# Quantum-Chemistry-Group-BNU/PyNQS

Measured on AMD Instinct MI355X. Metric: local energies/sec (whole node), higher is better.
Workload: dtype f64

## Files before the change

include/pynqs_amd.h:

```cpp
#ifndef PYNQS_AMD_H
#define PYNQS_AMD_H

#include <stdint.h>

#ifdef __cplusplus
extern "C" {
#endif

#define PYNQS_ABI_VERSION 1

#define PYNQS_OK 0
#define PYNQS_EINVAL (-1)
#define PYNQS_ELAUNCH (-2)
#define PYNQS_ELENGTH (-3)
#define PYNQS_EOVERFLOW (-4)

#define PYNQS_F32 0
#define PYNQS_F64 1

#define PYNQS_MAX_SORB_LEN 3
#define PYNQS_MAX_SORB 192
#define PYNQS_MAX_NELE 120
#define PYNQS_MAX_NVIR 120

int pynqs_abi_version(void);
const char *pynqs_last_error(void);

int64_t pynqs_num_sd(int sorb, int noA, int noB);

int pynqs_check_sorb(int sorb, int nele);

int pynqs_comb_hij_fused(const uint64_t *bra, int64_t nbatch, int sorb, int nele, int noA, int noB,
                         const void *h1e, const void *h2e, int dtype, uint64_t *comb, void *hmat,
                         void *stream);

int pynqs_comb(const uint64_t *bra, int64_t nbatch, int sorb, int noA, int noB, uint64_t *comb,
               double *comb_pm1, void *stream);

int pynqs_hij(const uint64_t *bra, int64_t n, const uint64_t *ket, int64_t m, int ket_is_3d,
              const void *h1e, const void *h2e, int dtype, int sorb, int nele, void *hmat, void *stream);

int pynqs_onv_to_pm1(const uint64_t *bra, int64_t n, int sorb, int dtype, void *out, void *stream);

int pynqs_pm01_to_onv(const uint8_t *occ, int64_t n, int sorb, uint64_t *out, void *stream);

int pynqs_wavefunction_lut(const uint64_t *keys, int64_t nkeys, const uint64_t *onv, int64_t n, int sorb,
                           int64_t *idx, uint8_t *mask, void *stream);

int pynqs_spin_flip_rand(const uint64_t *bra, int64_t n, int sorb, int noA, int noB, uint64_t seed,
                         uint64_t offset, uint64_t *out, void *stream);

int64_t pynqs_plan_bytes(int sorb, int dtype);
int pynqs_plan_build(const void *h1e, const void *h2e, int sorb, int dtype, void *plan, void *stream);

int pynqs_comb_hij_fused_plan(const uint64_t *bra, int64_t nbatch, int sorb, int nele, int noA, int noB,
                              const void *plan, int dtype, uint64_t *comb, void *hmat, void *stream);

int pynqs_eloc_sample_space(const uint64_t *bra, int64_t nbatch, int sorb, int nele, int noA, int noB,
                            const void *plan, const uint64_t *keys, int64_t nkeys, const double *wf,
                            int wf_is_complex, double *eloc, double *psi0, void *stream);

int64_t pynqs_hash_bytes(int64_t nkeys, int sorb);
int pynqs_hash_build(const uint64_t *keys, int64_t nkeys, int sorb, void *table, void *stream);
int pynqs_hash_lookup(const void *table, int64_t nkeys, const uint64_t *onv, int64_t n, int sorb, int64_t *idx,
                      uint8_t *mask, void *stream);
int pynqs_eloc_sample_space_hash(const uint64_t *bra, int64_t nbatch, int sorb, int nele, int noA, int noB,
                                 const void *plan, const void *table, int64_t nkeys, const double *wf,
                                 int wf_is_complex, double *eloc, double *psi0, void *stream);

int pynqs_eloc_sample_space_flip(const uint64_t *bra, int64_t nbatch, int sorb, int nele, int noA, int noB,
                                 const void *plan, const uint64_t *keys, int64_t nkeys, const double *wf,
                                 int wf_is_complex, const double *psi0, double *out, void *stream);
int pynqs_eloc_sample_space_hash_flip(const uint64_t *bra, int64_t nbatch, int sorb, int nele, int noA, int noB,
                                      const void *plan, const void *table, int64_t nkeys, const double *wf,
                                      int wf_is_complex, const double *psi0, double *out, void *stream);

int pynqs_eloc_sample_space_keys(const uint64_t *bra, int64_t nbatch, int sorb, int nele, int noA, int noB, const void *plan,
                                 const uint64_t *keys, int64_t nkeys, const double *wf, int wf_is_complex, int flip, double *eloc,
                                 double *psi0, void *stream);

int64_t pynqs_keys_index_bytes(int64_t nkeys, int sorb);
int64_t pynqs_keys_index_workspace(int64_t nkeys, int sorb);
int pynqs_keys_index_build(const uint64_t *keys, int64_t nkeys, int sorb, void *index, void *workspace, void *stream);
int pynqs_keys_index_density(const void *index, int64_t nkeys, int sorb, uint64_t *sum_sq, void *stream);
int pynqs_eloc_sample_space_indexed(const uint64_t *bra, int64_t nbatch, int sorb, int nele, int noA, int noB, const void *plan,
                                    const uint64_t *keys, int64_t nkeys, const void *index, const double *wf, int wf_is_complex,
                                    int flip, double *eloc, double *psi0, void *stream);

int pynqs_eloc_sample_space_form(int64_t nbatch, int sorb, int nele, int noA, int noB, int64_t nkeys, int hash, int64_t out[8]);
int pynqs_eloc_sample_space_keys_form(int64_t nbatch, int sorb, int64_t nkeys, int indexed, int64_t out[3]);

int64_t pynqs_unique_workspace(int64_t n);
int pynqs_unique_first(const uint64_t *onv, int64_t n, int sorb, void *workspace, int32_t *first, void *stream);

int pynqs_eloc_rbm_supported(int sorb, int nele, int noA, int noB, int nhidden);
int pynqs_eloc_rbm_form(int64_t nbatch, int sorb, int nele, int noA, int noB, int nhidden, int green);
int64_t pynqs_rbm_table_bytes(int sorb, int nhidden);
int pynqs_rbm_table_build(const double *weights, const double *hidden_bias, const double *visible_bias, int sorb,
                          int nhidden, void *table, void *stream);
int pynqs_eloc_rbm(const uint64_t *bra, int64_t nbatch, int sorb, int nele, int noA, int noB, const void *plan,
                   const void *rbm_table, int nhidden, double *eloc, double *psi, void *stream);
#define PYNQS_RBM_REAL 0
#define PYNQS_RBM_TANH 1
#define PYNQS_RBM_PHASE 2
int pynqs_eloc_rbm_flavour(const uint64_t *bra, int64_t nbatch, int sorb, int nele, int noA, int noB, const void *plan,
                           const void *rbm_table, int nhidden, int flavour, double *eloc, double *psi, void *stream);

int pynqs_eloc_rbm_flip_supported(int sorb, int nele, int noA, int noB, int nhidden);
int pynqs_eloc_rbm_flip_form(int64_t nbatch, int sorb, int nele, int noA, int noB, int nhidden);
int pynqs_eloc_rbm_signed(const uint64_t *bra, int64_t nbatch, int sorb, int nele, int noA, int noB, const void *plan,
                          const void *rbm_table, int nhidden, int flavour, double *eloc, double *psi, void *stream);
int pynqs_eloc_rbm_flip(const uint64_t *bra, int64_t nbatch, int sorb, int nele, int noA, int noB, const void *plan,
                        const void *rbm_table, const void *rbm_table_mirror, int nhidden, int flavour, double eta, double extra_norm,
                        const double *extra_norm_dev, double *eloc, double *psi, double *work, void *stream);

int pynqs_eloc_crbm_supported(int sorb, int nele, int noA, int noB, int nhidden);
int pynqs_eloc_crbm_form(int64_t nbatch, int sorb, int nele, int noA, int noB, int nhidden);
int64_t pynqs_crbm_table_bytes(int sorb, int nhidden);
int pynqs_crbm_table_build(const double *weights, const double *hidden_bias, const double *visible_bias, int sorb, int nhidden,
                           void *table, void *stream);
int pynqs_eloc_crbm(const uint64_t *bra, int64_t nbatch, int sorb, int nele, int noA, int noB, const void *plan,
                    const void *crbm_table, int nhidden, double log_scale, double *eloc, double *psi, void *stream);

int64_t pynqs_jastrow_table_bytes(int sorb);
int pynqs_jastrow_table_build(const double *jastrow, int sorb, void *table, void *stream);
int pynqs_eloc_jrbm_supported(int sorb, int nele, int noA, int noB, int nhidden);
int pynqs_eloc_jrbm_form(int64_t nbatch, int sorb, int nele, int noA, int noB, int nhidden);
int pynqs_eloc_jrbm(const uint64_t *bra, int64_t nbatch, int sorb, int nele, int noA, int noB, const void *plan,
                    const void *rbm_table, const void *jastrow_table, int nhidden, double *eloc, double *psi, void *stream);
int pynqs_eloc_jrbm_flip_supported(int sorb, int nele, int noA, int noB, int nhidden);
int pynqs_eloc_jrbm_flip_form(int64_t nbatch, int sorb, int nele, int noA, int noB, int nhidden);
int pynqs_eloc_jrbm_signed(const uint64_t *bra, int64_t nbatch, int sorb, int nele, int noA, int noB, const void *plan,
                           const void *rbm_table, const void *jastrow_table, int nhidden, double *eloc, double *psi, void *stream);
int pynqs_eloc_jrbm_flip(const uint64_t *bra, int64_t nbatch, int sorb, int nele, int noA, int noB, const void *plan,
                         const void *rbm_table, const void *jastrow_table, const void *rbm_table_mirror, const void *jastrow_table_mirror,
                         int nhidden, double eta, double extra_norm, const double *extra_norm_dev, double *eloc, double *psi, double *work,
                         void *stream);
int pynqs_jrbm_forward(const uint64_t *onv, int64_t n, int sorb, const double *weights, const double *hidden_bias,
                       const double *visible_bias, const double *jastrow, int nhidden, double *psi, void *stream);
int64_t pynqs_jastrow_grad_workspace(int64_t n, int sorb);
int pynqs_jastrow_grad(const uint64_t *onv, int64_t n, int sorb, const double *jastrow, const double *prob, const double *eloc,
                       const double *e_total, const double *pow, double *grad_jastrow, double *loss, void *workspace, void *stream);

int pynqs_gfmc_sample(const double *green, int64_t n, int64_t ncomb, const double *rand_num, const uint64_t *comb,
                      int sorb, int64_t *index, double *beta, uint64_t *x_new, void *stream);

int pynqs_green_rbm(const uint64_t *bra, int64_t nbatch, int sorb, int nele, int noA, int noB, const void *plan,
                    const void *rbm_table, int nhidden, int flavour, double lambda, double *eloc, double *psi, double *green,
                    uint8_t *clamped, void *stream);
int pynqs_gfmc_sample_rank(const double *green, int64_t n, const double *rand_num, const uint64_t *bra, int sorb, int nele,
                           int noA, int noB, int64_t *index, double *beta, uint64_t *x_new, void *stream);
int pynqs_green_jrbm(const uint64_t *bra, int64_t nbatch, int sorb, int nele, int noA, int noB, const void *plan,
                     const void *rbm_table, const void *jastrow_table, int nhidden, double lambda, double *eloc, double *psi,
                     double *green, uint8_t *clamped, void *stream);

int64_t pynqs_moments_workspace(void);
int pynqs_stats_finish(const double *moments, double inv_world, double counts, double *out5, void *stream);
int pynqs_weighted_moments(const double *x, int is_complex, const double *prob, int64_t n, void *workspace, void *stream);
int pynqs_weighted_moments_finish(const double *x, int is_complex, const double *prob, int64_t n, void *workspace, double inv_world,
                                  double counts, double *out5, void *stream);

int64_t pynqs_reduce_tiles(int64_t nbatch, int sorb, int nele, int noA, int noB);
int pynqs_reduce_count(const uint64_t *bra, int64_t nbatch, int sorb, int nele, int noA, int noB,
                       const void *plan, int dtype, double eps, uint32_t *tile_counts, void *stream);
int pynqs_reduce_emit(const uint64_t *bra, int64_t nbatch, int sorb, int nele, int noA, int noB,
                      const void *plan, int dtype, double eps, const int64_t *tile_offsets, int32_t *kept_col,
                      uint64_t *kept_onv, void *kept_h, void *stream);

int pynqs_reduce_count_sums(const uint64_t *bra, int64_t nbatch, int sorb, int nele, int noA, int noB,
                            const void *plan, int dtype, double eps, uint32_t *tile_counts, double *tile_sums,
                            void *stream);
int pynqs_reduce_sample(const uint64_t *bra, int64_t nbatch, int sorb, int nele, int noA, int noB, const void *plan,
                        int dtype, double eps, const int32_t *tile_draws, const int64_t *sample_offsets,
                        const double *walker_scale, uint64_t seed, int32_t *s_col, uint64_t *s_onv, void *s_h,
                        void *stream);

typedef struct pynqs_reduce_io {
  int64_t cap_doubles;
  int64_t cap_unique;
  int64_t dedup_slots;
  int32_t *rec_col;
  void *rec_w;
  uint64_t *rec_onv;
  int32_t *rec_link;
  int32_t *seg_count;
  int32_t *srec_col;
  void *srec_w;
  uint64_t *srec_onv;
  int32_t *srec_link;
  double *row_sum;
  void *dedup_table;
  uint64_t *uniq_onv;
  void *uniq_pm1;
  int32_t pm1_dtype;
  int32_t lut_is_hash;
  const void *lut_table;
  int64_t lut_nkeys;
  int32_t *counters;
  const uint64_t *seed_dev;
  void *row_cache;
  int32_t *uniq_parent;
  void *tile_scratch;
  int64_t tile_scratch_bytes;
  float *row_f32;
} pynqs_reduce_io;
int pynqs_reduce_onepass_geometry(int64_t nbatch, int sorb, int nele, int noA, int noB, int eps_sample, int64_t *out4);
int64_t pynqs_reduce_onepass_tile_scratch_bytes(int64_t nbatch, int sorb, int nele, int noA, int noB, int eps_sample);
int pynqs_reduce_onepass_list_capacity(int64_t nbatch, int sorb, int nele, int noA, int noB, int dtype, int eps_sample,
                                       int with_row_cache, int without_table, int64_t *cap_doubles);
int pynqs_reduce_onepass_wants_row_f32(int64_t nbatch, int sorb, int nele, int noA, int noB, int dtype, int eps_sample, int64_t cap_doubles,
                                       int with_tile_scratch ,
                                       int without_table );
int64_t pynqs_reduce_onepass_row_f32_elements(int64_t nbatch, int sorb, int nele, int noA, int noB);
int pynqs_reduce_onepass(const uint64_t *bra, int64_t nbatch, int sorb, int nele, int noA, int noB, const void *plan,
                         int dtype, double eps, int eps_sample, uint64_t seed, const pynqs_reduce_io *io, void *stream);
int pynqs_reduce_contract(int64_t nbatch, int sorb, int nele, int noA, int noB, int dtype, int eps_sample,
                          const pynqs_reduce_io *io, const double *psi_unique, const double *psi_table, int psi_is_complex,
                          int divide, double *eloc, double *psi_x, void *stream);

#define PYNQS_RBM_COMPLEX 4
int pynqs_rbm_forward(const uint64_t *onv, int64_t n, int sorb, const double *weights, const double *hidden_bias,
                      const double *visible_bias, int nhidden, int flavour, double *psi, void *stream);

int64_t pynqs_rbm_children_table_bytes(int64_t nwalkers, int sorb, int nhidden, int flavour);
int pynqs_rbm_children_prepare(const uint64_t *walkers, int64_t nwalkers, int sorb, const double *weights, const double *hidden_bias,
                               const double *visible_bias, int nhidden, int flavour, void *table, void *stream);
int pynqs_rbm_forward_children(const uint64_t *onv, int64_t n, const int32_t *count_dev, const int32_t *parent,
                               const uint64_t *walkers, int64_t nwalkers, const void *table, int sorb, const double *weights,
                               const double *hidden_bias, const double *visible_bias, int nhidden, int flavour, double *psi,
                               void *stream);
int pynqs_rbm_forward_children_supported(int sorb, int nhidden, int flavour);
int pynqs_rbm_children_prepare_stamped(const uint64_t *walkers, int64_t nwalkers, int sorb, const double *weights,
                                       const double *hidden_bias, const double *visible_bias, int nhidden, int flavour, uint64_t stamp,
                                       void *table, void *stream);
int pynqs_rbm_forward_children_stamped(const uint64_t *onv, int64_t n, const int32_t *count_dev, const int32_t *parent,
                                       const uint64_t *walkers, int64_t nwalkers, const void *table, int sorb, const double *weights,
                                       const double *hidden_bias, const double *visible_bias, int nhidden, int flavour, uint64_t stamp,
                                       double *psi, void *stream);

int64_t pynqs_rbm_grad_workspace(int64_t n, int sorb, int nhidden, int flavour);
int pynqs_rbm_grad(const uint64_t *onv, int64_t n, int sorb, const double *weights, const double *hidden_bias,
                   const double *visible_bias, int nhidden, int flavour, const double *prob, const double *eloc,
                   int eloc_is_complex, const double *e_total, const double *pow, double *grad_weights,
                   double *grad_hidden_bias, double *grad_visible_bias, double *loss, void *workspace, void *stream);
int pynqs_rbm_grad_loss(const uint64_t *onv, int64_t n, int sorb, const double *weights, const double *hidden_bias,
                        const double *visible_bias, int nhidden, int flavour, const double *prob, const double *eloc,
                        int eloc_is_complex, const double *e_total, const double *pow, double *grad_weights,
                        double *grad_hidden_bias, double *grad_visible_bias, double *loss, double *loss_copy, void *workspace,
                        void *stream);

#define PYNQS_SR_RHO 0
#define PYNQS_SR_RHS2 1
#define PYNQS_SR_DONE 2
#define PYNQS_SR_ITER 3
#define PYNQS_SR_TRUE2 4
#define PYNQS_SR_PAP 5
#define PYNQS_SR_CONVERGED 6
#define PYNQS_SR_BREAKDOWN 7
#define PYNQS_SR_NSCALARS 8
#define PYNQS_SR_CG_INIT 0
#define PYNQS_SR_CG_STEP 1
#define PYNQS_SR_CG_RESIDUAL 2
int64_t pynqs_rbm_sr_workspace(int64_t n, int sorb, int nhidden, int flavour);
int pynqs_rbm_sr_prepare(const uint64_t *onv, int64_t n, int sorb, const double *weights, const double *hidden_bias, int nhidden,
                         int flavour, const double *prob, void *workspace, double *obar, void *stream);
int pynqs_rbm_sr_matvec(const uint64_t *onv, int64_t n, int sorb, int nhidden, int flavour, const double *prob, const void *workspace,
                        const double *obar, const double *v, double *y, void *stream);
int pynqs_rbm_sr_cg_step(int mode, int64_t np, double *y, const double *rhs, double *d, double *r, double *p, double *scalars,
                         double inv_world, double diag_shift, double tol, void *stream);
int64_t pynqs_jrbm_sr_workspace(int64_t n, int sorb, int nhidden);
int pynqs_jrbm_sr_prepare(const uint64_t *onv, int64_t n, int sorb, const double *weights, const double *hidden_bias, int nhidden,
                          const double *prob, void *workspace, double *obar, void *stream);
int pynqs_jrbm_sr_matvec(const uint64_t *onv, int64_t n, int sorb, int nhidden, const double *prob, const void *workspace,
                         const double *obar, const double *v, double *y, void *stream);

#define PYNQS_MCMC_ACCEPT_KEY 0x243F6A8885A308D3ull
int pynqs_mcmc_rbm_supported(int sorb, int nhidden, int flavour);
int pynqs_mcmc_rbm(uint64_t *states, int64_t nchains, int sorb, int noA, int noB, const void *table, int nhidden, int flavour,
                   uint64_t seed, uint64_t chain_base, uint64_t t0, int nsteps, int every, uint64_t *records, int64_t *n_accept,
                   double *lnpsi, void *stream);
int pynqs_mcmc_jrbm_supported(int sorb, int nhidden);
int pynqs_mcmc_jrbm_form(int sorb, int nhidden);
int pynqs_mcmc_jrbm(uint64_t *states, int64_t nchains, int sorb, int noA, int noB, const void *rbm_table, const void *jastrow_table,
                    int nhidden, uint64_t seed, uint64_t chain_base, uint64_t t0, int nsteps, int every, uint64_t *records,
                    int64_t *n_accept, double *lnpsi, void *stream);
int pynqs_mcmc_accept(uint64_t *states, double *psi, const uint64_t *proposals, const double *psi_proposals, int64_t nchains,
                      int sorb, int is_complex, uint64_t seed, uint64_t chain_base, uint64_t t, uint64_t *record_row,
                      int64_t *n_accept, void *stream);

int pynqs_rdm_scatter(const uint64_t *bra, int64_t nbatch, int sorb, int nele, int noA, int noB, const double *w, const double *ratio,
                      int is_complex, double *rdm1, double *rdm2, void *stream);
int pynqs_rdm_rbm_supported(int sorb, int nele, int noA, int noB, int nhidden);
int64_t pynqs_rdm_rbm_workspace(int64_t nbatch, int sorb, int nhidden);
int pynqs_rdm_rbm(const uint64_t *bra, int64_t nbatch, int sorb, int nele, int noA, int noB, const double *w, const void *rbm_table,
                  int nhidden, void *workspace, double *rdm1, double *rdm2, void *stream);
int pynqs_rdm_jrbm_supported(int sorb, int nele, int noA, int noB, int nhidden);
int64_t pynqs_rdm_jrbm_workspace(int64_t nbatch, int sorb, int nhidden);
int pynqs_rdm_jrbm(const uint64_t *bra, int64_t nbatch, int sorb, int nele, int noA, int noB, const double *w, const void *rbm_table,
                   const void *jastrow_table, int nhidden, void *workspace, double *rdm1, double *rdm2, void *stream);

#ifdef __cplusplus
}
#endif
#endif
```

pynqs_amd/_native.py:

```python
from __future__ import annotations

import ctypes as C
import os

_HERE = os.path.dirname(os.path.abspath(__file__))
LIB_PATH = os.environ.get("PYNQS_AMD_LIB") or os.path.join(_HERE, "csrc", "libpynqs_amd.so")

PYNQS_F32, PYNQS_F64 = 0, 1
RBM_REAL, RBM_TANH, RBM_PHASE, RBM_COMPLEX = 0, 1, 2, 4
OK, EINVAL, ELAUNCH, ELENGTH, EOVERFLOW = 0, -1, -2, -3, -4

_i64, _int, _vp, _dbl = C.c_int64, C.c_int, C.c_void_p, C.c_double

SIGNATURES = {
    "pynqs_abi_version": (_int, []),
    "pynqs_last_error": (C.c_char_p, []),
    "pynqs_num_sd": (_i64, [_int, _int, _int]),
    "pynqs_check_sorb": (_int, [_int, _int]),
    "pynqs_comb_hij_fused": (_int, [_vp, _i64, _int, _int, _int, _int, _vp, _vp, _int, _vp, _vp, _vp]),
    "pynqs_comb": (_int, [_vp, _i64, _int, _int, _int, _vp, _vp, _vp]),
    "pynqs_hij": (_int, [_vp, _i64, _vp, _i64, _int, _vp, _vp, _int, _int, _int, _vp, _vp]),
    "pynqs_onv_to_pm1": (_int, [_vp, _i64, _int, _int, _vp, _vp]),
    "pynqs_pm01_to_onv": (_int, [_vp, _i64, _int, _vp, _vp]),
    "pynqs_wavefunction_lut": (_int, [_vp, _i64, _vp, _i64, _int, _vp, _vp, _vp]),
    "pynqs_spin_flip_rand": (_int, [_vp, _i64, _int, _int, _int, C.c_uint64, C.c_uint64, _vp, _vp]),
    "pynqs_plan_bytes": (_i64, [_int, _int]),
    "pynqs_plan_build": (_int, [_vp, _vp, _int, _int, _vp, _vp]),
    "pynqs_comb_hij_fused_plan": (_int, [_vp, _i64, _int, _int, _int, _int, _vp, _int, _vp, _vp, _vp]),
    "pynqs_eloc_sample_space": (_int, [_vp, _i64, _int, _int, _int, _int, _vp, _vp, _i64, _vp, _int, _vp, _vp, _vp]),
    "pynqs_hash_bytes": (_i64, [_i64, _int]),
    "pynqs_hash_build": (_int, [_vp, _i64, _int, _vp, _vp]),
    "pynqs_hash_lookup": (_int, [_vp, _i64, _vp, _i64, _int, _vp, _vp, _vp]),
    "pynqs_unique_workspace": (_i64, [_i64]),
    "pynqs_unique_first": (_int, [_vp, _i64, _int, _vp, _vp, _vp]),
    "pynqs_eloc_sample_space_hash": (_int, [_vp, _i64, _int, _int, _int, _int, _vp, _vp, _i64, _vp, _int, _vp, _vp, _vp]),
    "pynqs_eloc_sample_space_flip": (_int, [_vp, _i64, _int, _int, _int, _int, _vp, _vp, _i64, _vp, _int, _vp, _vp, _vp]),
    "pynqs_eloc_sample_space_hash_flip": (_int, [_vp, _i64, _int, _int, _int, _int, _vp, _vp, _i64, _vp, _int, _vp, _vp, _vp]),
    "pynqs_eloc_sample_space_keys": (_int, [_vp, _i64, _int, _int, _int, _int, _vp, _vp, _i64, _vp, _int, _int, _vp, _vp, _vp]),
    "pynqs_keys_index_bytes": (_i64, [_i64, _int]),
    "pynqs_keys_index_workspace": (_i64, [_i64, _int]),
    "pynqs_keys_index_build": (_int, [_vp, _i64, _int, _vp, _vp, _vp]),
    "pynqs_keys_index_density": (_int, [_vp, _i64, _int, _vp, _vp]),
    "pynqs_eloc_sample_space_indexed": (_int, [_vp, _i64, _int, _int, _int, _int, _vp, _vp, _i64, _vp, _vp, _int, _int, _vp, _vp, _vp]),
    "pynqs_eloc_sample_space_form": (_int, [_i64, _int, _int, _int, _int, _i64, _int, C.POINTER(_i64)]),
    "pynqs_eloc_sample_space_keys_form": (_int, [_i64, _int, _i64, _int, C.POINTER(_i64)]),
    "pynqs_eloc_rbm_supported": (_int, [_int, _int, _int, _int, _int]),
    "pynqs_eloc_rbm_form": (_int, [_i64, _int, _int, _int, _int, _int, _int]),
    "pynqs_rbm_table_bytes": (_i64, [_int, _int]),
    "pynqs_rbm_table_build": (_int, [_vp, _vp, _vp, _int, _int, _vp, _vp]),
    "pynqs_eloc_rbm": (_int, [_vp, _i64, _int, _int, _int, _int, _vp, _vp, _int, _vp, _vp, _vp]),
    "pynqs_eloc_rbm_flavour": (_int, [_vp, _i64, _int, _int, _int, _int, _vp, _vp, _int, _int, _vp, _vp, _vp]),
    "pynqs_eloc_rbm_flip_supported": (_int, [_int, _int, _int, _int, _int]),
    "pynqs_eloc_rbm_flip_form": (_int, [_i64, _int, _int, _int, _int, _int]),
    "pynqs_eloc_rbm_signed": (_int, [_vp, _i64, _int, _int, _int, _int, _vp, _vp, _int, _int, _vp, _vp, _vp]),
    "pynqs_eloc_rbm_flip": (_int, [_vp, _i64, _int, _int, _int, _int, _vp, _vp, _vp, _int, _int, _dbl, _dbl, _vp, _vp, _vp, _vp, _vp]),
    "pynqs_eloc_crbm_supported": (_int, [_int, _int, _int, _int, _int]),
    "pynqs_eloc_crbm_form": (_int, [_i64, _int, _int, _int, _int, _int]),
    "pynqs_crbm_table_bytes": (_i64, [_int, _int]),
    "pynqs_crbm_table_build": (_int, [_vp, _vp, _vp, _int, _int, _vp, _vp]),
    "pynqs_eloc_crbm": (_int, [_vp, _i64, _int, _int, _int, _int, _vp, _vp, _int, _dbl, _vp, _vp, _vp]),
    "pynqs_gfmc_sample": (_int, [_vp, _i64, _i64, _vp, _vp, _int, _vp, _vp, _vp, _vp]),
    "pynqs_green_rbm": (_int, [_vp, _i64, _int, _int, _int, _int, _vp, _vp, _int, _int, _dbl, _vp, _vp, _vp, _vp, _vp]),
    "pynqs_gfmc_sample_rank": (_int, [_vp, _i64, _vp, _vp, _int, _int, _int, _int, _vp, _vp, _vp, _vp]),
    "pynqs_moments_workspace": (_i64, []),
    "pynqs_stats_finish": (_int, [_vp, _dbl, _dbl, _vp, _vp]),
    "pynqs_weighted_moments": (_int, [_vp, _int, _vp, _i64, _vp, _vp]),
    "pynqs_weighted_moments_finish": (_int, [_vp, _int, _vp, _i64, _vp, _dbl, _dbl, _vp, _vp]),
    "pynqs_reduce_tiles": (_i64, [_i64, _int, _int, _int, _int]),
    "pynqs_reduce_count": (_int, [_vp, _i64, _int, _int, _int, _int, _vp, _int, _dbl, _vp, _vp]),
    "pynqs_reduce_count_sums": (_int, [_vp, _i64, _int, _int, _int, _int, _vp, _int, _dbl, _vp, _vp, _vp]),
    "pynqs_reduce_sample": (_int, [_vp, _i64, _int, _int, _int, _int, _vp, _int, _dbl, _vp, _vp, _vp, C.c_uint64, _vp, _vp, _vp, _vp]),
    "pynqs_reduce_emit": (_int, [_vp, _i64, _int, _int, _int, _int, _vp, _int, _dbl, _vp, _vp, _vp, _vp, _vp]),
}



class ReduceIO(C.Structure):
    _fields_ = [("cap_doubles", _i64), ("cap_unique", _i64), ("dedup_slots", _i64),
                ("rec_col", _vp), ("rec_w", _vp), ("rec_onv", _vp), ("rec_link", _vp), ("seg_count", _vp),
                ("srec_col", _vp), ("srec_w", _vp), ("srec_onv", _vp), ("srec_link", _vp), ("row_sum", _vp),
                ("dedup_table", _vp), ("uniq_onv", _vp), ("uniq_pm1", _vp), ("pm1_dtype", C.c_int32), ("lut_is_hash", C.c_int32),
                ("lut_table", _vp), ("lut_nkeys", _i64), ("counters", _vp), ("seed_dev", _vp), ("row_cache", _vp), ("uniq_parent", _vp),
                ("tile_scratch", _vp), ("tile_scratch_bytes", _i64), ("row_f32", _vp)]


SIGNATURES.update({
    "pynqs_reduce_onepass_geometry": (_int, [_i64, _int, _int, _int, _int, _int, C.POINTER(_i64)]),
    "pynqs_reduce_onepass_tile_scratch_bytes": (_i64, [_i64, _int, _int, _int, _int, _int]),
    "pynqs_reduce_onepass_list_capacity": (_int, [_i64, _int, _int, _int, _int, _int, _int, _int, _int, C.POINTER(_i64)]),
    "pynqs_reduce_onepass_wants_row_f32": (_int, [_i64, _int, _int, _int, _int, _int, _int, _i64, _int, _int]),
    "pynqs_reduce_onepass_row_f32_elements": (_i64, [_i64, _int, _int, _int, _int]),
    "pynqs_reduce_onepass": (_int, [_vp, _i64, _int, _int, _int, _int, _vp, _int, _dbl, _int, C.c_uint64, C.POINTER(ReduceIO), _vp]),
    "pynqs_rbm_forward": (_int, [_vp, _i64, _int, _vp, _vp, _vp, _int, _int, _vp, _vp]),
    "pynqs_rbm_children_table_bytes": (_i64, [_i64, _int, _int, _int]),
    "pynqs_rbm_children_prepare": (_int, [_vp, _i64, _int, _vp, _vp, _vp, _int, _int, _vp, _vp]),
    "pynqs_rbm_forward_children": (_int, [_vp, _i64, _vp, _vp, _vp, _i64, _vp, _int, _vp, _vp, _vp, _int, _int, _vp, _vp]),
    "pynqs_rbm_forward_children_supported": (_int, [_int, _int, _int]),
    "pynqs_rbm_children_prepare_stamped": (_int, [_vp, _i64, _int, _vp, _vp, _vp, _int, _int, C.c_uint64, _vp, _vp]),
    "pynqs_rbm_forward_children_stamped": (_int, [_vp, _i64, _vp, _vp, _vp, _i64, _vp, _int, _vp, _vp, _vp, _int, _int, C.c_uint64, _vp, _vp]),
    "pynqs_rbm_grad_workspace": (_i64, [_i64, _int, _int, _int]),
    "pynqs_rbm_grad": (_int, [_vp, _i64, _int, _vp, _vp, _vp, _int, _int, _vp, _vp, _int, _vp, _vp, _vp, _vp, _vp, _vp, _vp, _vp]),
    "pynqs_rbm_grad_loss": (_int, [_vp, _i64, _int, _vp, _vp, _vp, _int, _int, _vp, _vp, _int, _vp, _vp, _vp, _vp, _vp, _vp, _vp, _vp, _vp]),
    "pynqs_reduce_contract": (_int, [_i64, _int, _int, _int, _int, _int, _int, C.POINTER(ReduceIO), _vp, _vp, _int, _int, _vp, _vp, _vp]),    "pynqs_mcmc_rbm_supported": (_int, [_int, _int, _int]),
    "pynqs_mcmc_rbm": (_int, [_vp, _i64, _int, _int, _int, _vp, _int, _int, C.c_uint64, C.c_uint64, C.c_uint64, _int, _int, _vp, _vp, _vp, _vp]),
    "pynqs_rbm_sr_workspace": (_i64, [_i64, _int, _int, _int]),
    "pynqs_rbm_sr_prepare": (_int, [_vp, _i64, _int, _vp, _vp, _int, _int, _vp, _vp, _vp, _vp]),
    "pynqs_rbm_sr_matvec": (_int, [_vp, _i64, _int, _int, _int, _vp, _vp, _vp, _vp, _vp, _vp]),
    "pynqs_rbm_sr_cg_step": (_int, [_int, _i64, _vp, _vp, _vp, _vp, _vp, _vp, _dbl, _dbl, _dbl, _vp]),
    "pynqs_jrbm_sr_workspace": (_i64, [_i64, _int, _int]),
    "pynqs_jrbm_sr_prepare": (_int, [_vp, _i64, _int, _vp, _vp, _int, _vp, _vp, _vp, _vp]),
    "pynqs_jrbm_sr_matvec": (_int, [_vp, _i64, _int, _int, _vp, _vp, _vp, _vp, _vp, _vp]),
    "pynqs_mcmc_accept": (_int, [_vp, _vp, _vp, _vp, _i64, _int, _int, C.c_uint64, C.c_uint64, C.c_uint64, _vp, _vp, _vp]),
    "pynqs_rdm_scatter": (_int, [_vp, _i64, _int, _int, _int, _int, _vp, _vp, _int, _vp, _vp, _vp]),
    "pynqs_rdm_rbm_supported": (_int, [_int, _int, _int, _int, _int]),
    "pynqs_rdm_rbm_workspace": (_i64, [_i64, _int, _int]),
    "pynqs_rdm_rbm": (_int, [_vp, _i64, _int, _int, _int, _int, _vp, _vp, _int, _vp, _vp, _vp, _vp]),
    "pynqs_rdm_jrbm_supported": (_int, [_int, _int, _int, _int, _int]),
    "pynqs_rdm_jrbm_workspace": (_i64, [_i64, _int, _int]),
    "pynqs_rdm_jrbm": (_int, [_vp, _i64, _int, _int, _int, _int, _vp, _vp, _vp, _int, _vp, _vp, _vp, _vp]),
    "pynqs_jastrow_table_bytes": (_i64, [_int]),
    "pynqs_jastrow_table_build": (_int, [_vp, _int, _vp, _vp]),
    "pynqs_eloc_jrbm_supported": (_int, [_int, _int, _int, _int, _int]),
    "pynqs_eloc_jrbm_form": (_int, [_i64, _int, _int, _int, _int, _int]),
    "pynqs_eloc_jrbm": (_int, [_vp, _i64, _int, _int, _int, _int, _vp, _vp, _vp, _int, _vp, _vp, _vp]),
    "pynqs_eloc_jrbm_flip_supported": (_int, [_int, _int, _int, _int, _int]),
    "pynqs_eloc_jrbm_flip_form": (_int, [_i64, _int, _int, _int, _int, _int]),
    "pynqs_eloc_jrbm_signed": (_int, [_vp, _i64, _int, _int, _int, _int, _vp, _vp, _vp, _int, _vp, _vp, _vp]),
    "pynqs_eloc_jrbm_flip": (_int, [_vp, _i64, _int, _int, _int, _int, _vp, _vp, _vp, _vp, _vp, _int, _dbl, _dbl, _vp, _vp, _vp, _vp, _vp]),
    "pynqs_green_jrbm": (_int, [_vp, _i64, _int, _int, _int, _int, _vp, _vp, _vp, _int, _dbl, _vp, _vp, _vp, _vp, _vp]),
    "pynqs_jrbm_forward": (_int, [_vp, _i64, _int, _vp, _vp, _vp, _vp, _int, _vp, _vp]),
    "pynqs_jastrow_grad_workspace": (_i64, [_i64, _int]),
    "pynqs_mcmc_jrbm_supported": (_int, [_int, _int]),
    "pynqs_mcmc_jrbm_form": (_int, [_int, _int]),
    "pynqs_mcmc_jrbm": (_int, [_vp, _i64, _int, _int, _int, _vp, _vp, _int, C.c_uint64, C.c_uint64, C.c_uint64, _int, _int, _vp, _vp, _vp, _vp]),
    "pynqs_jastrow_grad": (_int, [_vp, _i64, _int, _vp, _vp, _vp, _vp, _vp, _vp, _vp, _vp, _vp]),
})

_lib = None


class NativeLibraryError(RuntimeError):
    pass


def lib() -> C.CDLL:
    global _lib
    if _lib is None:
        if not os.path.exists(LIB_PATH):
            raise NativeLibraryError(
                f"{LIB_PATH} not found: build the HIP extension first (python -c 'import __graft_entry__ as g; g.build()'). "
                "pynqs_amd has no CPU fallback."
            )
        try:
            l = C.CDLL(LIB_PATH)
        except OSError as e:
            raise NativeLibraryError(f"cannot load {LIB_PATH}: {e}") from e
        for name, (res, args) in SIGNATURES.items():
            f = getattr(l, name)
            f.restype = res
            f.argtypes = args
        if l.pynqs_abi_version() != 1:
            raise NativeLibraryError("libpynqs_amd.so ABI version mismatch")
        _lib = l
    return _lib


def check(rc: int, what: str) -> None:
    if rc == OK:
        return
    msg = lib().pynqs_last_error().decode(errors="replace")
    if rc == ELENGTH:
        raise ValueError(msg)
    if rc == EOVERFLOW:
        raise OverflowError(msg)
    raise RuntimeError(f"{what}: {msg} (code {rc})")
```

pynqs_amd/csrc/kernels_gfmc.hip:

```cpp
#include "detcore.h"
#include "launch.h"

namespace pynqs {

constexpr int kGfmcMaxTiles = 1024;

__device__ __forceinline__ double wave_incl_scan(double v, int lane) {
#pragma unroll
  for (int d = 1; d < 64; d <<= 1) {
    const double o = __shfl_up(v, d);
    if (lane >= d) v += o;
  }
  return v;
}

template <int LEN, bool FROM_RANK>
__global__ __launch_bounds__(kBlock) void gfmc_sample_kernel(const double *__restrict__ gk, int64_t m, uint32_t tile, uint32_t ntiles,
                                                             const double *__restrict__ rnd, const uint64_t *__restrict__ comb, SDParams p,
                                                             int64_t *__restrict__ index, double *__restrict__ beta,
                                                             uint64_t *__restrict__ x_new) {
  __shared__ double tsum[kGfmcMaxTiles];
  __shared__ double s_target, s_before;
  __shared__ uint32_t s_tile;
  const int64_t walker = blockIdx.x;
  const int tid = threadIdx.x, lane = tid & 63, wave = tid >> 6;
  const double *__restrict__ row = gk + walker * m;
  for (uint32_t t = wave; t < ntiles; t += kBlock / 64) {
    const int64_t c0 = (int64_t)t * tile, c1 = min(c0 + (int64_t)tile, m);
    double acc = 0.0;
    for (int64_t c = c0 + lane; c < c1; c += 64) acc += row[c];
#pragma unroll
    for (int d = 32; d > 0; d >>= 1) acc += __shfl_xor(acc, d);
    if (lane == 0) tsum[t] = acc;
  }
  __syncthreads();
  if (wave == 0) {
    constexpr int kPer = kGfmcMaxTiles / 64;
    double loc[kPer], s = 0.0;
#pragma unroll
    for (int i = 0; i < kPer; ++i) {
      const uint32_t t = lane * kPer + i;
      loc[i] = t < ntiles ? tsum[t] : 0.0;
      s += loc[i];
    }
    const double incl = wave_incl_scan(s, lane);
    const double total = __shfl(incl, 63);
    const double target = rnd[walker] * total;
    const double lower = __shfl_up(incl, 1);
    double before = lane ? lower : 0.0;
    uint32_t mine = 0xffffffffu, last = 0xffffffffu;
    double mine_before = 0.0, last_before = 0.0;
#pragma unroll
    for (int i = 0; i < kPer; ++i) {
      const uint32_t t = lane * kPer + i;
      if (loc[i] > 0.0) {
        if (mine == 0xffffffffu && before + loc[i] >= target) { mine = t; mine_before = before; }
        last = t; last_before = before;
      }
      before += loc[i];
    }
    const uint64_t have = __ballot(mine != 0xffffffffu);
    const uint64_t any = __ballot(last != 0xffffffffu);
    const int src = have ? __ffsll((long long)have) - 1 : any ? 63 - __clzll((long long)any) : 0;
    if (lane == src) {
      s_tile = !(target > 0.0) ? 0xffffffffu : have ? mine : any ? last : 0xffffffffu;
      s_before = have ? mine_before : last_before;
      s_target = target;
    }
    if (lane == 0) beta[walker] = total;
  }
  __syncthreads();
  if (wave == 0) {
    const uint32_t t = s_tile;
    const double target = s_target;
    double run = s_before;
    const int64_t c0 = (int64_t)t * tile, c1 = min(c0 + (int64_t)tile, m);
    int64_t found = -1, last_pos = -1;
    if (t == 0xffffffffu) found = 0;
    for (int64_t c = c0; c < c1 && found < 0; c += 64) {
      const double v = c + lane < c1 ? row[c + lane] : 0.0;
      const double incl = wave_incl_scan(v, lane) + run;
      const uint64_t pos = __ballot(v > 0.0);
      const uint64_t hit = pos & __ballot(incl >= target);
      if (hit) found = c + __ffsll((long long)hit) - 1;
      if (pos) last_pos = c + 63 - __clzll((long long)pos);
      run = __shfl(incl, 63);
    }
    if (found < 0) found = last_pos >= 0 ? last_pos : 0;
    if (lane == 0) index[walker] = found;
    if constexpr (FROM_RANK) {
      if (lane == 0) {
        uint64_t x[LEN];
#pragma unroll
        for (int i = 0; i < LEN; ++i) x[i] = comb[walker * LEN + i];
        if (found > 0) excite_by_rank<LEN>(x, (uint32_t)(found - 1), p);
#pragma unroll
        for (int i = 0; i < LEN; ++i) x_new[walker * LEN + i] = x[i];
      }
    } else {
      if (lane < LEN) x_new[walker * LEN + lane] = comb[(walker * m + found) * LEN + lane];
    }
  }
}

}

using namespace pynqs;

template <bool FROM_RANK>
static int gfmc_sample_impl(const double *green, int64_t n, int64_t ncomb, const double *rand_num, const uint64_t *comb, int sorb,
                            const SDParams &p, int64_t *index, double *beta, uint64_t *x_new, void *stream) {
  pynqs::DeviceScope device_scope_(green);
  if (n < 0 || ncomb < 1 || sorb < 1 || sorb > kMaxSorb) return set_error(PYNQS_EINVAL, "bad n / ncomb / sorb");
  if (n == 0) return PYNQS_OK;
  if (!green || !rand_num || !comb || !index || !beta || !x_new) return set_error(PYNQS_EINVAL, "null pointer");
  if (n > 0x7fffffffll) return set_error(PYNQS_EINVAL, "n too large for one launch");
  uint32_t tile = 256;
  while ((ncomb + tile - 1) / tile > kGfmcMaxTiles) tile *= 2;
  const uint32_t ntiles = (uint32_t)((ncomb + tile - 1) / tile);
  const int len = (sorb - 1) / 64 + 1;
  hipStream_t st = (hipStream_t)stream;
  DISPATCH_LEN(len, hipLaunchKernelGGL((gfmc_sample_kernel<LEN, FROM_RANK>), dim3((uint32_t)n), dim3(kBlock), 0, st, green, ncomb, tile, ntiles,
                                       rand_num, comb, p, index, beta, x_new));
  return check_launch("gfmc_sample");
}

extern "C" int pynqs_gfmc_sample(const double *green, int64_t n, int64_t ncomb, const double *rand_num, const uint64_t *comb, int sorb,
                                 int64_t *index, double *beta, uint64_t *x_new, void *stream) {
  SDParams p = {};
  return gfmc_sample_impl<false>(green, n, ncomb, rand_num, comb, sorb, p, index, beta, x_new, stream);
}

extern "C" int pynqs_gfmc_sample_rank(const double *green, int64_t n, const double *rand_num, const uint64_t *bra, int sorb, int nele,
                                      int noA, int noB, int64_t *index, double *beta, uint64_t *x_new, void *stream) {
  SDParams p;
  if (!make_sd_params(sorb, nele, noA, noB, &p)) return set_error(PYNQS_EINVAL, "bad sorb/noA/noB");
  return gfmc_sample_impl<true>(green, n, (int64_t)p.nsd + 1, rand_num, bra, sorb, p, index, beta, x_new, stream);
}

namespace pynqs {

constexpr int kMomentBlocks = 128;

__device__ __forceinline__ void stats_finish(const double *m, double inv_world, double counts, double *__restrict__ out) {
  const double re = m[0] * inv_world, im = m[1] * inv_world, m2 = m[2] * inv_world, ps = m[3] * inv_world;
  double var = m2 - (re * re + im * im) * (2.0 - ps);
  var = var > 0.0 ? var : 0.0;
  const double sd = sqrt(var);
  out[0] = re; out[1] = im; out[2] = var; out[3] = sd; out[4] = sd / sqrt(counts);
}

template <bool CPLX, bool FINISH>
__global__ __launch_bounds__(kBlock) void moments_kernel(const double *__restrict__ x, const double *__restrict__ prob, int64_t n,
                                                         double *__restrict__ out, unsigned int *__restrict__ done, double inv_world,
                                                         double counts, double *__restrict__ out5) {
  __shared__ double red[4][kBlock / 64];
  __shared__ bool last;
  const int tid = threadIdx.x, lane = tid & 63, wave = tid >> 6;
  double s[4] = {0.0, 0.0, 0.0, 0.0};
  for (int64_t i = (int64_t)blockIdx.x * kBlock + tid; i < n; i += (int64_t)gridDim.x * kBlock) {
    const double p = prob[i];
    const double re = CPLX ? x[2 * i] : x[i], im = CPLX ? x[2 * i + 1] : 0.0;
    s[0] += p * re; s[1] += p * im; s[2] += p * (re * re + im * im); s[3] += p;
  }
#pragma unroll
  for (int k = 0; k < 4; ++k) {
#pragma unroll
    for (int d = 32; d > 0; d >>= 1) s[k] += __shfl_xor(s[k], d);
    if (lane == 0) red[k][wave] = s[k];
  }
  __syncthreads();
  if (tid < 4) {
    double t = 0.0;
    for (int w = 0; w < kBlock / 64; ++w) t += red[tid][w];
    out[4 * (1 + blockIdx.x) + tid] = t;
  }
  __threadfence();
  __syncthreads();
  if (tid == 0) last = atomicAdd(done, 1u) == gridDim.x - 1;
  __syncthreads();
  if (last) {
    __threadfence();
    if (tid < 4) {
      double t = 0.0;
      for (unsigned b = 0; b < gridDim.x; ++b) t += out[4 * (1 + b) + tid];
      out[tid] = t;
      if constexpr (FINISH) red[0][tid] = t;
    }
    if (tid == 0) *done = 0;
    if constexpr (FINISH) {
      __syncthreads();
      if (tid == 0) stats_finish(&red[0][0], inv_world, counts, out5);
    }
  }
}

__global__ void stats_finish_kernel(const double *__restrict__ m, double inv_world, double counts, double *__restrict__ out) {
  stats_finish(m, inv_world, counts, out);
}

}

extern "C" int pynqs_stats_finish(const double *moments, double inv_world, double counts, double *out5, void *stream) {
  pynqs::DeviceScope device_scope_(moments);
  if (!moments || !out5 || !(counts > 0.0)) return set_error(PYNQS_EINVAL, "bad arguments");
  hipLaunchKernelGGL(stats_finish_kernel, dim3(1), dim3(1), 0, (hipStream_t)stream, moments, inv_world, counts, out5);
  return check_launch("stats_finish");
}

extern "C" int64_t pynqs_moments_workspace(void) { return 8 * 4 * (pynqs::kMomentBlocks + 1) + 8; }

static int weighted_moments_launch(const double *x, int is_complex, const double *prob, int64_t n, void *workspace, bool finish, double inv_world,
                                   double counts, double *out5, void *stream) {
  pynqs::DeviceScope device_scope_(x);
  if (n < 0) return set_error(PYNQS_EINVAL, "bad n");
  if (!workspace || (n > 0 && (!x || !prob))) return set_error(PYNQS_EINVAL, "null pointer");
  if (finish && (!out5 || !(counts > 0.0))) return set_error(PYNQS_EINVAL, "bad arguments");
  double *out = (double *)workspace;
  unsigned int *done = (unsigned int *)(out + 4 * (kMomentBlocks + 1));
  int64_t blocks = (n + kBlock - 1) / kBlock;
  if (blocks > kMomentBlocks) blocks = kMomentBlocks;
  if (blocks < 1) blocks = 1;
  hipStream_t st = (hipStream_t)stream;
#define PYNQS_MK(C, F) \
  hipLaunchKernelGGL((moments_kernel<C, F>), dim3((uint32_t)blocks), dim3(kBlock), 0, st, x, prob, n, out, done, inv_world, counts, out5)
  if (finish) { if (is_complex) PYNQS_MK(true, true); else PYNQS_MK(false, true); }
  else { if (is_complex) PYNQS_MK(true, false); else PYNQS_MK(false, false); }
#undef PYNQS_MK
  return check_launch("weighted_moments");
}

extern "C" int pynqs_weighted_moments(const double *x, int is_complex, const double *prob, int64_t n, void *workspace, void *stream) {
  return weighted_moments_launch(x, is_complex, prob, n, workspace, false, 1.0, 1.0, nullptr, stream);
}

extern "C" int pynqs_weighted_moments_finish(const double *x, int is_complex, const double *prob, int64_t n, void *workspace, double inv_world,
                                             double counts, double *out5, void *stream) {
  return weighted_moments_launch(x, is_complex, prob, n, workspace, true, inv_world, counts, out5, stream);
}
```

pynqs_amd/csrc/kernels_rbm_grad.hip:

```cpp
#include "detcore.h"
#include "launch.h"
#include "rbm_math.h"

namespace pynqs {

constexpr int kGradWalkers = 32;
constexpr int kGradHidden = 32;

template <int LEN, bool CPLX, int B>
__global__ __launch_bounds__(B) void rbm_grad_partial_kernel(const uint64_t *__restrict__ onv, int64_t n, int sorb, int H,
                                                                  const double *__restrict__ W, const double *__restrict__ hb,
                                                                  const double *__restrict__ vb, const double *__restrict__ prob,
                                                                  const double *__restrict__ eloc, bool eloc_cplx,
                                                                  const double *__restrict__ e_total, const double *__restrict__ pw,
                                                                  double *__restrict__ partial, int64_t stride) {
  constexpr int C = CPLX ? 2 : 1;
  __shared__ uint64_t xs[kGradWalkers][LEN];
  __shared__ double tc[kGradWalkers][kGradHidden + 1][C];
  __shared__ double cf[kGradWalkers][C];
  constexpr int NQ = B / kGradWalkers;
  const int tid = threadIdx.x, w = tid % kGradWalkers, q = tid / kGradWalkers;
  const int64_t i = (int64_t)blockIdx.x * kGradWalkers + w;
  const bool valid = i < n;
  const int64_t row = valid ? i : n - 1;
  uint64_t ket[LEN];
#pragma unroll
  for (int k = 0; k < LEN; ++k) ket[k] = onv[row * LEN + k];
  double fr = 0.0, fi = 0.0;
  if (valid) {
    const double pr = prob[i], c = pw ? pw[i] : 1.0;
    const double er = eloc_cplx ? eloc[2 * i] : eloc[i], ei = eloc_cplx ? eloc[2 * i + 1] : 0.0;
    const double tr = e_total[0], ti = eloc_cplx ? e_total[1] : 0.0;
    fr = pr * (er - tr * c);
    fi = pr * (ei - ti * c);
  }
  if (q == 0) {
#pragma unroll
    for (int k = 0; k < LEN; ++k) xs[w][k] = ket[k];
    cf[w][0] = fr;
    if constexpr (CPLX) cf[w][1] = -fi;
  }
  double *__restrict__ out = partial + (int64_t)blockIdx.x * stride;
  double lre = 0.0, lim = 0.0;
  const int SP = sorb + 1;
  for (int h0 = 0; h0 < H; h0 += kGradHidden) {
    constexpr int HC = kGradHidden / NQ;
    double tr[HC], ti[HC];
#pragma unroll
    for (int j = 0; j < HC; ++j) {
      const int h = min(h0 + HC * q + j, H - 1);
      tr[j] = CPLX ? hb[2 * h] : hb[h];
      ti[j] = CPLX ? hb[2 * h + 1] : 0.0;
    }
    for (int o = 0; o < sorb; ++o) {
      const double x = pm1_of<LEN>(ket, o);
#pragma unroll
      for (int j = 0; j < HC; ++j) {
        const int h = min(h0 + HC * q + j, H - 1);
        if constexpr (CPLX) {
          tr[j] = fma(x, W[((size_t)h * sorb + o) * 2], tr[j]);
          ti[j] = fma(x, W[((size_t)h * sorb + o) * 2 + 1], ti[j]);
        } else {
          tr[j] = fma(x, W[(size_t)h * sorb + o], tr[j]);
        }
      }
    }
    if (h0) __syncthreads();
#pragma unroll
    for (int j = 0; j < HC; ++j) {
      const int hh = HC * q + j;
      const bool live = h0 + hh < H;
      const double ax = fabs(tr[j]), e = exp(-2.0 * ax), s = tr[j] < 0.0 ? -1.0 : 1.0;
      double yr, yi = 0.0;
      if constexpr (CPLX) {
        double sn, cs;
        sincos_mod(2.0 * ti[j], sn, cs);
        const double den = fma(2.0 * e, cs, fma(e, e, 1.0));
        yr = s * (1.0 - e * e) / den;
        yi = 2.0 * e * sn / den;
        if (live) {
          const double u = fma(e, cs, 1.0), v = -s * e * sn;
          lre += ax + 0.5 * log(u * u + v * v);
          lim += s * ti[j] + atan2(v, u);
        }
        tc[w][hh][0] = live ? yr * fr + yi * fi : 0.0;
        tc[w][hh][1] = live ? yi * fr - yr * fi : 0.0;
      } else {
        yr = s * (1.0 - e) / (1.0 + e);
        if (live) lre += ax + log1p(e);
        tc[w][hh][0] = live ? yr * fr : 0.0;
      }
    }
    __syncthreads();
    const int nout = min(kGradHidden, H - h0) * SP;
    for (int k = tid; k < nout; k += B) {
      const int hh = k / SP, o = k - hh * SP;
      double ar = 0.0, ai = 0.0;
      if (o < sorb) {
        const int word = o >> 6, bit = o & 63;
#pragma unroll 8
        for (int v = 0; v < kGradWalkers; ++v) {
          const bool up = (xs[v][word] >> bit) & 1ull;
          const double a = tc[v][hh][0];
          ar += up ? a : -a;
          if constexpr (CPLX) { const double b = tc[v][hh][1]; ai += up ? b : -b; }
        }
      } else {
#pragma unroll 8
        for (int v = 0; v < kGradWalkers; ++v) {
          ar += tc[v][hh][0];
          if constexpr (CPLX) ai += tc[v][hh][1];
        }
      }
      const int64_t at = (int64_t)(h0 + hh) * SP + o;
      out[C * at] = ar;
      if constexpr (CPLX) out[C * at + 1] = ai;
    }
  }
  const int64_t off_vb = (int64_t)H * SP;
  for (int o = tid; o < sorb; o += B) {
    const int word = o >> 6, bit = o & 63;
    double ar = 0.0, ai = 0.0;
#pragma unroll 4
    for (int v = 0; v < kGradWalkers; ++v) {
      const bool up = (xs[v][word] >> bit) & 1ull;
      ar += up ? cf[v][0] : -cf[v][0];
      if constexpr (CPLX) ai += up ? cf[v][1] : -cf[v][1];
    }
    out[C * (off_vb + o)] = ar;
    if constexpr (CPLX) out[C * (off_vb + o) + 1] = ai;
  }
  if (vb && q == 0) {
    for (int o = 0; o < sorb; ++o) {
      const double x = pm1_of<LEN>(ket, o);
      lre = fma(x, CPLX ? vb[2 * o] : vb[o], lre);
      if constexpr (CPLX) lim = fma(x, vb[2 * o + 1], lim);
    }
  }
  __syncthreads();
  static_assert(NQ * kGradWalkers * 2 <= kGradWalkers * (kGradHidden + 1) * C && kGradHidden % NQ == 0, "B: 256 or 512");
  double *lr = &tc[0][0][0];
  lr[(q * kGradWalkers + w) * 2] = lre;
  lr[(q * kGradWalkers + w) * 2 + 1] = lim;
  __syncthreads();
  if (tid < 64) {
    double l = 0.0;
    if (q == 0) {
      double re = 0.0, im = 0.0;
#pragma unroll
      for (int k = 0; k < NQ; ++k) { re += lr[(k * kGradWalkers + w) * 2]; im += lr[(k * kGradWalkers + w) * 2 + 1]; }
      im -= 6.283185307179586476925 * rint(im * 0.15915494309189533577);
      l = valid ? 2.0 * (re * fr + im * fi) : 0.0;
    }
#pragma unroll
    for (int d = 32; d > 0; d >>= 1) l += __shfl_xor(l, d);
    if (tid == 0) out[C * (off_vb + sorb)] = l;
  }
}

template <bool CPLX>
__global__ __launch_bounds__(kBlock) void rbm_grad_reduce_kernel(const double *__restrict__ partial, int64_t stride, int ngroups, int sorb, int H,
                                                                 double *__restrict__ gw, double *__restrict__ ghb, double *__restrict__ gvb,
                                                                 double *__restrict__ loss, double *__restrict__ loss_copy) {
  constexpr int C = CPLX ? 2 : 1;
  constexpr int NS = kBlock / 64;
  __shared__ double part[NS][64][2];
  const int SP = sorb + 1;
  const int64_t nout = (int64_t)H * SP + sorb + 1;
  const int lane = threadIdx.x & 63, slice = threadIdx.x >> 6;
  const int64_t k = (int64_t)blockIdx.x * 64 + lane;
  const int per = (ngroups + NS - 1) / NS, g_lo = min(slice * per, ngroups), g_hi = min(g_lo + per, ngroups);
  double re = 0.0, im = 0.0;
  if (k < nout) {
    constexpr int RU = 16;
    for (int g0 = g_lo; g0 < g_hi; g0 += RU) {
      double vr[RU], vi[RU];
#pragma unroll
      for (int u = 0; u < RU; ++u) {
        const bool in = g0 + u < g_hi;
        vr[u] = in ? partial[(int64_t)(g0 + u) * stride + C * k] : 0.0;
        vi[u] = CPLX && in ? partial[(int64_t)(g0 + u) * stride + C * k + 1] : 0.0;
      }
#pragma unroll
      for (int u = 0; u < RU; ++u) { re += vr[u]; im += vi[u]; }
    }
  }
  part[slice][lane][0] = re;
  part[slice][lane][1] = im;
  __syncthreads();
  if (slice != 0 || k >= nout) return;
  re = 0.0; im = 0.0;
#pragma unroll
  for (int sl = 0; sl < NS; ++sl) { re += part[sl][lane][0]; im += part[sl][lane][1]; }
  if (k == nout - 1) {
    if (loss) loss[0] = re;
    if (loss_copy) loss_copy[0] = re;
    return;
  }
  double *dst;
  int64_t at;
  if (k < (int64_t)H * SP) {
    const int64_t h = k / SP;
    const int o = (int)(k - h * SP);
    if (o < sorb) { dst = gw; at = h * sorb + o; }
    else { dst = ghb; at = h; }
  } else {
    dst = gvb; at = k - (int64_t)H * SP;
  }
  if (!dst) return;
  dst[C * at] = 2.0 * re;
  if constexpr (CPLX) dst[C * at + 1] = -2.0 * im;
}

static inline int64_t grad_stride(int sorb, int H, bool cplx) {
  return ((int64_t)H * (sorb + 1) + sorb + 1) * (cplx ? 2 : 1);
}

}

using namespace pynqs;

extern "C" int64_t pynqs_rbm_grad_workspace(int64_t n, int sorb, int nhidden, int flavour) {
  if (n < 0 || sorb < 1 || sorb > kMaxSorb || nhidden < 1 || (flavour != PYNQS_RBM_REAL && flavour != PYNQS_RBM_COMPLEX)) return -1;
  const int64_t groups = (n + kGradWalkers - 1) / kGradWalkers;
  return groups * grad_stride(sorb, nhidden, flavour == PYNQS_RBM_COMPLEX) * 8;
}

static int grad_block() {
  static const int b = getenv("PYNQS_RBM_GRAD_BLOCK") ? atoi(getenv("PYNQS_RBM_GRAD_BLOCK")) : 512;
  return b == 256 ? 256 : 512;
}

extern "C" int pynqs_rbm_grad_loss(const uint64_t *onv, int64_t n, int sorb, const double *weights, const double *hidden_bias,
                                   const double *visible_bias, int nhidden, int flavour, const double *prob, const double *eloc,
                                   int eloc_is_complex, const double *e_total, const double *pow, double *grad_weights, double *grad_hidden_bias,
                                   double *grad_visible_bias, double *loss, double *loss_copy, void *workspace, void *stream) {
  pynqs::DeviceScope device_scope_(onv);
  if (n < 0 || n > 0x7fffffffll * kGradWalkers || sorb < 1 || sorb > kMaxSorb || nhidden < 1) return set_error(PYNQS_EINVAL, "bad n/sorb/nhidden");
  if (flavour != PYNQS_RBM_REAL && flavour != PYNQS_RBM_COMPLEX) return set_error(PYNQS_EINVAL, "rbm_grad: flavour must be PYNQS_RBM_REAL or PYNQS_RBM_COMPLEX");
  if (!weights || !hidden_bias || !grad_weights || !grad_hidden_bias || (n > 0 && (!onv || !prob || !eloc || !e_total || !workspace)))
    return set_error(PYNQS_EINVAL, "null pointer");
  const bool cplx = flavour == PYNQS_RBM_COMPLEX;
  const int len = (sorb - 1) / 64 + 1;
  const int64_t groups = (n + kGradWalkers - 1) / kGradWalkers, stride = grad_stride(sorb, nhidden, cplx);
  hipStream_t st = (hipStream_t)stream;
  double *partial = (double *)workspace;
  if (groups > 0) {
    const bool wide = grad_block() == 512;
#define PYNQS_RG(C, B)                                                                                                                         \
  hipLaunchKernelGGL((rbm_grad_partial_kernel<LEN, C, B>), dim3((uint32_t)groups), dim3(B), 0, st, onv, n, sorb, nhidden, weights, hidden_bias, \
                     visible_bias, prob, eloc, eloc_is_complex != 0, e_total, pow, partial, stride)
    DISPATCH_LEN(len, {
      if (cplx) { if (wide) PYNQS_RG(true, 512); else PYNQS_RG(true, 256); }
      else { if (wide) PYNQS_RG(false, 512); else PYNQS_RG(false, 256); }
    });
#undef PYNQS_RG
  }
  const int64_t nout = (int64_t)nhidden * (sorb + 1) + sorb + 1;
  const uint32_t g2 = (uint32_t)((nout + 63) / 64);
  if (cplx)
    hipLaunchKernelGGL((rbm_grad_reduce_kernel<true>), dim3(g2), dim3(kBlock), 0, st, partial, stride, (int)groups, sorb, nhidden, grad_weights,
                       grad_hidden_bias, grad_visible_bias, loss, loss_copy);
  else
    hipLaunchKernelGGL((rbm_grad_reduce_kernel<false>), dim3(g2), dim3(kBlock), 0, st, partial, stride, (int)groups, sorb, nhidden, grad_weights,
                       grad_hidden_bias, grad_visible_bias, loss, loss_copy);
  return check_launch("rbm_grad");
}

extern "C" int pynqs_rbm_grad(const uint64_t *onv, int64_t n, int sorb, const double *weights, const double *hidden_bias,
                              const double *visible_bias, int nhidden, int flavour, const double *prob, const double *eloc,
                              int eloc_is_complex, const double *e_total, const double *pow, double *grad_weights, double *grad_hidden_bias,
                              double *grad_visible_bias, double *loss, void *workspace, void *stream) {
  return pynqs_rbm_grad_loss(onv, n, sorb, weights, hidden_bias, visible_bias, nhidden, flavour, prob, eloc, eloc_is_complex, e_total, pow,
                             grad_weights, grad_hidden_bias, grad_visible_bias, loss, nullptr, workspace, stream);
}
```

pynqs_amd/csrc/kernels_reduce_onepass.hip:

```cpp
#include "detcore.h"
#include "launch.h"
#include "plan.h"
#include "plan_dev.h"
#include "plan_tiles.h"
#include "reduce_common.h"
#include "reduce_list.h"

namespace pynqs {




template <int LEN, typename T, bool SAMPLED>
struct KeepSink {
  T eps;
  uint32_t chunk, nchunks, tS;
  int64_t seg_base;
  volatile uint32_t *run;
  WinnerList wl;
  uint32_t *bufc;
  T *bufh;
  volatile uint32_t *dstat;
  double *tsum;
  uint32_t *kept_total;
  const SDParams *p;
  const LdsLayout *L;
  const Walker<LEN> *wk;
  OnepassOut<T> o;
  uint32_t tile;
  double sub;

  __device__ __forceinline__ int32_t record(int64_t g, uint32_t col, T h, const uint64_t (&ket)[LEN], bool &unlisted) const {
    o.rec_col[g] = (int32_t)col;
    o.rec_w[g] = h;
    if (o.rec_onv) {
#pragma unroll
      for (int i = 0; i < LEN; ++i) o.rec_onv[g * LEN + i] = ket[i];
    }
    const int32_t link = resolve_amplitude<LEN, T>(o, wl, ket, col, unlisted);
    o.rec_link[g] = link;
    return link;
  }

  __device__ __forceinline__ void fixed_slot(uint32_t slot, uint32_t col, T h, const uint64_t (&ket)[LEN]) {
    const T a = fabs(h);
    if (!(a >= eps)) {
      if constexpr (SAMPLED) sub += (double)a;
      return;
    }
    bool unlisted;
    const int32_t link = record(seg_base + slot, col, h, ket, unlisted);
    if (unlisted) {
      const int32_t r = atomicAdd(o.counters, 1);
      if (assign_row<LEN, T>(o, (uint32_t)link, r, ket) && o.uniq_pm1) {
        for (int j = 0; j < p->sorb; ++j) {
          const bool occ = (ket[j >> 6] >> (j & 63)) & 1ull;
          if (o.pm1_f32) reinterpret_cast<float *>(o.uniq_pm1)[(size_t)r * p->sorb + j] = occ ? 1.0f : -1.0f;
          else reinterpret_cast<double *>(o.uniq_pm1)[(size_t)r * p->sorb + j] = occ ? 1.0 : -1.0;
        }
      }
    }
  }

  __device__ __forceinline__ uint32_t advance(uint32_t total) const {
    const int lane = threadIdx.x & 63;
    const int leader = __ffsll((long long)__ballot(1)) - 1;
    uint32_t before = 0;
    if (lane == leader) { before = *run; *run = before + total; }
    return __shfl(before, leader);
  }

  __device__ __forceinline__ void one(uint32_t col, T h, const uint64_t (&ket)[LEN]) {
    if (tile == 0) { fixed_slot(col == 0 ? 0u : 1u + (threadIdx.x & 63u), col, h, ket); return; }
    if (tile <= tS) {
      const uint32_t r0 = (chunk + (tile - 1) * nchunks) * kSinglesPerTile;
      fixed_slot(kFixedHead + (tile - 1) * kSinglesPerTile + (col - 1 - r0), col, h, ket);
      return;
    }
    const T a = fabs(h);
    const bool k = a >= eps;
    if constexpr (SAMPLED) { if (!k) sub += (double)a; }
    const uint64_t m = __ballot(k);
    if (!m) return;
    const uint32_t before = advance((uint32_t)__popcll(m));
    if (k) {
      const uint32_t at = before + __popcll(m & ((1ull << (threadIdx.x & 63)) - 1ull));
      bufc[at] = col;
      bufh[at] = h;
    }
  }
  __device__ __forceinline__ void two(uint32_t c0, T h0, const uint64_t (&)[LEN], uint32_t c1, T h1, const uint64_t (&)[LEN]) {
    const T a0 = fabs(h0), a1 = fabs(h1);
    const bool a = a0 >= eps, b = a1 >= eps;
    if constexpr (SAMPLED) sub += (a ? 0.0 : (double)a0) + (b ? 0.0 : (double)a1);
    const uint64_t ma = __ballot(a), mb = __ballot(b);
    if (!(ma | mb)) return;
    const uint32_t before = advance((uint32_t)(__popcll(ma) + __popcll(mb)));
    const uint64_t below = (1ull << (threadIdx.x & 63)) - 1ull;
    const uint32_t mine = before + __popcll(ma & below) + __popcll(mb & below);
    if (a) { bufc[mine] = c0; bufh[mine] = h0; }
    if (b) { bufc[mine + (a ? 1 : 0)] = c1; bufh[mine + (a ? 1 : 0)] = h1; }
  }
  __device__ __forceinline__ void pair(uint32_t col, T h0, T h1, const uint64_t (&k0)[LEN], const uint64_t (&k1)[LEN]) {
    two(col, h0, k0, col + 1, h1, k1);
  }

  __device__ __forceinline__ uint32_t lookback(uint32_t d, uint32_t c) const {
    const int lane = threadIdx.x & 63;
    if (d == 0 || (o.debug & 4u)) {
      if (lane == 0) dstat[d] = kStatP | c;
      return 0;
    }
    if (lane == 0) dstat[d] = kStatA | c;
    uint32_t excl = 0;
    int32_t top = (int32_t)d - 1;
    for (;;) {
      const int32_t idx = top - lane;
      const uint32_t s = idx >= 0 ? dstat[idx] : kStatP;
      const uint64_t ready = __ballot(s != 0u);
      const uint64_t isP = __ballot((s & kStatP) != 0u);
      const int fp = isP ? __ffsll((long long)isP) - 1 : 64;
      const uint64_t need = fp >= 63 ? ~0ull : ((2ull << fp) - 1ull);
      if ((ready & need) != need) {
        __builtin_amdgcn_s_sleep(1);
        continue;
      }
      excl += op_wave_sum(lane <= fp ? (s & kStatMask) : 0u);
      if (fp < 64) break;
      top -= 64;
    }
    if (lane == 0) dstat[d] = kStatP | (excl + c);
    return excl;
  }

  __device__ __forceinline__ void flush() {
    if (tile == 0xffffffffu) return;
    const int lane = threadIdx.x & 63;
    if constexpr (SAMPLED) {
      const double s = op_wave_sum(sub);
      if (lane == 0) tsum[tile] = s;
    }
    wave_sync();
    if (tile <= tS) return;
    const uint32_t c = *run;
    const uint32_t excl = lookback(tile - 1 - tS, c);
    if (lane == 0 && c) atomicMax(kept_total, excl + c);
    for (uint32_t i0 = 0; i0 < c; i0 += 64) {
      const uint32_t i = i0 + lane;
      const bool act = i < c && excl + i < o.cap_d;
      bool unlisted = false;
      int32_t link = -1;
      uint64_t ket[LEN];
#pragma unroll
      for (int w = 0; w < LEN; ++w) ket[w] = 0ull;
      if (act) {
        const uint32_t col = bufc[i];
        const Excitation x = decode(col - 1, *p, *L);
        make_ket<LEN>(*wk, x, ket);
        link = record(seg_base + o.fixed + excl + i, col, bufh[i], ket, unlisted);
      }
      if (__ballot(unlisted)) allocate_now<LEN, T>(o, p->sorb, unlisted, (uint32_t)link, ket);
    }
  }
  __device__ __forceinline__ void tile_begin(uint32_t t) {
    flush();
    tile = t;
    sub = 0.0;
    if ((threadIdx.x & 63) == 0) *run = 0u;
    __builtin_amdgcn_wave_barrier();
  }
};


template <int LEN, typename T>
struct DrawSink {
  T eps;
  DrawLds S;
  const SDParams *p;
  const LdsLayout *L;
  const Walker<LEN> *wk;
  const uint32_t *dinfo;
  double scale;
  uint64_t key;
  int64_t sbase;
  OnepassOut<T> o;
  WinnerList wl;
  uint32_t tile;

  __device__ __forceinline__ void entry(uint32_t idx, uint32_t col, T h, double incl) const {
    S.prefix[idx] = incl;
    S.cs[idx] = col | (h < T(0) ? 0x80000000u : 0u);
  }
  __device__ __forceinline__ double width(T h) const {
    const T a = fabs(h);
    return a >= eps ? 0.0 : (double)a;
  }
  __device__ __forceinline__ void one(uint32_t col, T h, const uint64_t (&)[LEN]) const {
    const int lane = threadIdx.x & 63;
    uint64_t m = __ballot(1);
    const double w = width(h);
    while (m) {
      const int b = __ffsll((long long)m) - 1;
      m &= m - 1;
      if (lane == b) {
        const uint32_t idx = *S.ncols;
        const double incl = *S.run + w;
        entry(idx, col, h, incl);
        *S.ncols = idx + 1;
        *S.run = incl;
      }
      __builtin_amdgcn_wave_barrier();
    }
  }
  __device__ __forceinline__ void pair(uint32_t col, T h0, T h1, const uint64_t (&)[LEN], const uint64_t (&)[LEN]) const {
    const int lane = threadIdx.x & 63;
    const uint32_t nact = (uint32_t)__popcll(__ballot(1));
    const double w0 = width(h0), w1 = width(h1);
    const double incl = op_scan(w0 + w1, lane);
    const uint32_t base = *S.ncols;
    const double run = *S.run;
    entry(base + 2 * lane, col, h0, run + incl - w1);
    entry(base + 2 * lane + 1, col + 1, h1, run + incl);
    const double total = __shfl(incl, (int)nact - 1);
    __builtin_amdgcn_wave_barrier();
    if (lane == 0) { *S.ncols = base + 2 * nact; *S.run = run + total; }
    __builtin_amdgcn_wave_barrier();
  }
  __device__ __forceinline__ void two(uint32_t c0, T h0, const uint64_t (&)[LEN], uint32_t c1, T h1, const uint64_t (&)[LEN]) const {
    const int lane = threadIdx.x & 63;
    const double w0 = width(h0), w1 = width(h1);
    const double i0 = op_scan(w0, lane), t0 = __shfl(i0, 63);
    const double i1 = op_scan(w1, lane), t1 = __shfl(i1, 63);
    const uint32_t base = *S.ncols;
    const double run = *S.run;
    entry(base + lane, c0, h0, run + i0);
    entry(base + 64 + lane, c1, h1, run + t0 + i1);
    __builtin_amdgcn_wave_barrier();
    if (lane == 0) { *S.ncols = base + 128; *S.run = run + t0 + t1; }
    __builtin_amdgcn_wave_barrier();
  }

  __device__ __forceinline__ void flush() {
    if (tile == 0xffffffffu) return;
    const int lane = threadIdx.x & 63;
    const uint32_t info = dinfo[tile];
    const uint32_t draws = info & 0xffffu;
    const uint32_t ncols = *S.ncols;
    const double total = *S.run;
    if (draws == 0 || ncols == 0 || !(total > 0.0)) return;
    for (uint32_t k = lane; k < draws; k += 64) {
      const uint64_t r = op_mix64(key ^ op_mix64(((uint64_t)tile << 32) | k));
      const double target = (double)(r >> 11) * 0x1.0p-53 * total;
      uint32_t lo = 0, hi = ncols;
      while (lo < hi) {
        const uint32_t mid = (lo + hi) >> 1;
        if (S.prefix[mid] > target) hi = mid; else lo = mid + 1;
      }
      if (lo >= ncols) lo = ncols - 1;
      while (lo > 0 && !(S.prefix[lo] > S.prefix[lo - 1])) --lo;
      atomicAdd(&S.hits[lo], 1u);
    }
    __builtin_amdgcn_wave_barrier();
    int64_t pos = sbase + (info >> 16);
    for (uint32_t i0 = 0; i0 < ncols; i0 += 64) {
      const uint32_t idx = i0 + lane;
      const uint32_t hc = idx < ncols ? S.hits[idx] : 0u;
      const uint64_t m = __ballot(hc != 0u);
      bool unlisted = false;
      int32_t link = -1;
      uint64_t ket[LEN];
#pragma unroll
      for (int w = 0; w < LEN; ++w) ket[w] = 0ull;
      if (hc) {
        const uint32_t e = S.cs[idx], col = e & 0x7fffffffu;
        const int64_t at = pos + __popcll(m & ((1ull << lane) - 1ull));
        if (col == 0) {
#pragma unroll
          for (int i = 0; i < LEN; ++i) ket[i] = wk->w[i];
        } else {
          const Excitation x = decode(col - 1, *p, *L);
          make_ket<LEN>(*wk, x, ket);
        }
        o.srec_col[at] = (int32_t)col;
        const double v = scale * (double)hc;
        o.srec_w[at] = (T)((e >> 31) ? -v : v);
        if (o.srec_onv) {
#pragma unroll
          for (int i = 0; i < LEN; ++i) o.srec_onv[at * LEN + i] = ket[i];
        }
        link = resolve_amplitude<LEN, T>(o, wl, ket, col, unlisted);
        o.srec_link[at] = link;
      }
      if (__ballot(unlisted)) allocate_now<LEN, T>(o, p->sorb, unlisted, (uint32_t)link, ket);
      pos += __popcll(m);
    }
  }
  __device__ __forceinline__ bool skip_tile(uint32_t t) const { return (dinfo[t] & 0xffffu) == 0u; }
  __device__ __forceinline__ void tile_begin(uint32_t t) {
    flush();
    tile = t;
    if ((dinfo[t] & 0xffffu) == 0u) return;
    const int lane = threadIdx.x & 63;
    __builtin_amdgcn_wave_barrier();
    for (int i = lane; i < kOneTileCols; i += 64) S.hits[i] = 0u;
    if (lane == 0) { *S.ncols = 0u; *S.run = 0.0; }
    __builtin_amdgcn_wave_barrier();
  }
};

__host__ __device__ inline size_t onepass_lds(const SDParams &p, size_t esz, uint32_t max_tiles, bool sampled, uint32_t wl_cap) {
  size_t b = (lds_bytes(p, esz) + 15) & ~(size_t)15;
  b += ((size_t)max_tiles * 4 + 15) & ~(size_t)15;
  if (sampled) {
    b += (size_t)max_tiles * 8;
    b += ((size_t)max_tiles * 4 + 15) & ~(size_t)15;
    b += (kBlock / 64) * kDrawLdsPerWave;
  }
  return b + (size_t)wl_cap * 8;
}

__host__ inline uint32_t winner_list_cap(int eps_sample) {
  uint32_t c = eps_sample > 256 ? (uint32_t)eps_sample : 256u;
  c = (c + 63u) & ~63u;
  return c > 2048u ? 2048u : c;
}

template <int LEN, typename T, bool SAMPLED>
__global__ __launch_bounds__(kBlock) void reduce_onepass_kernel(const uint64_t *__restrict__ bra, SDParams p, PlanLayout pl, uint32_t nchunks,
                                                                uint32_t chunk_len, uint32_t max_tiles, const T *__restrict__ plan, T eps,
                                                                uint32_t nsample, uint64_t seed, uint32_t wl_cap, OnepassOut<T> o) {
  extern __shared__ __attribute__((aligned(16))) unsigned char smem[];
  __shared__ uint32_t next_tile, kept_total, wl_n;
  __shared__ int32_t wl_base;
  __shared__ uint32_t wave_run[kBlock / 64];
  __shared__ double s_part[kBlock / 64 + 1];
  __shared__ uint32_t s_parti[kBlock / 64 + 1];
  uint64_t walker;
  uint32_t chunk;
  map_workgroup(nchunks, false, walker, chunk);
  o.parent = (int32_t)walker;
  const uint64_t slot = walker * nchunks + chunk;
  const int tid = threadIdx.x, lane = tid & 63, wave = tid >> 6;
  const int64_t seg_base = (int64_t)slot * ((int64_t)o.fixed + o.cap_d);
  if (tid == 0) { next_tile = 0; kept_total = 0; wl_n = 0; }
  unsigned char *extra = smem + ((lds_bytes(p, sizeof(T)) + 15) & ~(size_t)15);
  volatile uint32_t *dstat = reinterpret_cast<volatile uint32_t *>(extra);
  extra += ((size_t)max_tiles * 4 + 15) & ~(size_t)15;
  double *tsum = reinterpret_cast<double *>(extra);
  uint32_t *dinfo = reinterpret_cast<uint32_t *>(extra + (SAMPLED ? (size_t)max_tiles * 8 : 0));
  WinnerList wl;
  wl.n = &wl_n;
  wl.cap = wl_cap;
  wl.slot = reinterpret_cast<uint32_t *>(smem + onepass_lds(p, sizeof(T), max_tiles, SAMPLED, 0));
  wl.col = wl.slot + wl_cap;
  for (uint32_t i = tid; i < max_tiles; i += kBlock) {
    dstat[i] = 0u;
    if constexpr (SAMPLED) { tsum[i] = 0.0; dinfo[i] = 0u; }
  }
  for (uint32_t i = tid; i < o.fixed; i += kBlock) o.rec_col[seg_base + i] = -1;
  if constexpr (SAMPLED) {
    for (uint32_t i = tid; i < nsample; i += kBlock) o.srec_col[(int64_t)walker * nsample + i] = -1;
  }
  Walker<LEN> wk;
  load_walker<LEN>(bra + walker * LEN, wk);
  const LdsLayout L = carve_lds(smem, p);
  const int nocc = build_walker_tables<LEN>(wk, p, L);

  const uint32_t tS_all = (p.d1 + kSinglesPerTile - 1) / kSinglesPerTile;
  const uint32_t tS = tS_all > chunk ? (tS_all - chunk + nchunks - 1) / nchunks : 0;
  T *quarter = reinterpret_cast<T *>(L.scratch) + wave * (kDiagTile / 4);
  {
    KeepSink<LEN, T, SAMPLED> sink;
    sink.eps = eps; sink.chunk = chunk; sink.nchunks = nchunks; sink.tS = tS; sink.seg_base = seg_base;
    sink.run = wave_run + wave; sink.wl = wl;
    sink.bufh = quarter;
    sink.bufc = reinterpret_cast<uint32_t *>(quarter + kOneTileCols);
    sink.dstat = dstat; sink.tsum = tsum; sink.kept_total = &kept_total;
    sink.p = &p; sink.L = &L; sink.wk = &wk; sink.o = o; sink.tile = 0xffffffffu; sink.sub = 0.0;
    visit_tiles<LEN, T>(p, pl, L, nocc, plan, wk, nchunks, chunk, chunk_len, 0u, &next_tile, sink);
    sink.flush();
  }
  flush_winner_list<LEN, T>(o, wl, &wl_base, p, L, wk);
  if (tid == 0) {
    o.seg_count[slot] = (int32_t)kept_total;
    if (kept_total > o.cap_d) {
      atomicOr(reinterpret_cast<unsigned int *>(o.counters + 1), 1u);
      atomicMax(o.counters + 2, (int32_t)kept_total);
    }
  }
  if constexpr (SAMPLED) {
    const uint32_t per = (max_tiles + kBlock - 1) / kBlock;
    const uint32_t b0 = min((uint32_t)tid * per, max_tiles), b1 = min(b0 + per, max_tiles);
    double local = 0.0;
    for (uint32_t i = b0; i < b1; ++i) local += tsum[i];
    double incl = op_scan(local, lane);
    if (lane == 63) s_part[wave] = incl;
    __syncthreads();
    double before = 0.0, total = 0.0;
    for (int w = 0; w < kBlock / 64; ++w) {
      if (w < wave) before += s_part[w];
      total += s_part[w];
    }
    double run = before + incl - local;
    for (uint32_t i = b0; i < b1; ++i) { run += tsum[i]; tsum[i] = run; }
    __syncthreads();
    const double Srow = total;
    if (tid == 0 && o.row_sum) o.row_sum[walker] = Srow;
    const uint64_t key = op_mix64((o.seed_dev ? seed + *o.seed_dev : seed) ^ op_mix64(slot));
    if (Srow > 0.0) {
      for (uint32_t k = tid; k < nsample; k += kBlock) {
        const uint64_t r = op_mix64(key ^ op_mix64(0xffffffff00000000ull | k));
        const double target = (double)(r >> 11) * 0x1.0p-53 * Srow;
        uint32_t lo = 0, hi = max_tiles;
        while (lo < hi) {
          const uint32_t mid = (lo + hi) >> 1;
          if (tsum[mid] > target) hi = mid; else lo = mid + 1;
        }
        if (lo >= max_tiles) lo = max_tiles - 1;
        while (lo > 0 && !(tsum[lo] > tsum[lo - 1])) --lo;
        atomicAdd(&dinfo[lo], 1u);
      }
    }
    __syncthreads();
    uint32_t lsum = 0;
    for (uint32_t i = b0; i < b1; ++i) lsum += dinfo[i];
    uint32_t iscan = lsum;
#pragma unroll
    for (int d = 1; d < 64; d <<= 1) {
      const uint32_t ov = __shfl_up(iscan, d);
      if (lane >= d) iscan += ov;
    }
    if (lane == 63) s_parti[wave] = iscan;
    __syncthreads();
    uint32_t ibefore = 0;
    for (int w = 0; w < wave; ++w) ibefore += s_parti[w];
    uint32_t off = ibefore + iscan - lsum;
    for (uint32_t i = b0; i < b1; ++i) {
      const uint32_t c = dinfo[i];
      dinfo[i] = (off << 16) | c;
      off += c;
    }
    if (tid == 0) next_tile = 0;
    __syncthreads();
    unsigned char *mine = reinterpret_cast<unsigned char *>(dinfo) + (((size_t)max_tiles * 4 + 15) & ~(size_t)15) + (size_t)wave * kDrawLdsPerWave;
    DrawLds S;
    S.prefix = reinterpret_cast<double *>(mine);
    S.run = reinterpret_cast<volatile double *>(mine + (size_t)kOneTileCols * 8);
    S.cs = reinterpret_cast<uint32_t *>(mine + (size_t)kOneTileCols * 8 + 8);
    S.hits = S.cs + kOneTileCols;
    S.ncols = reinterpret_cast<volatile uint32_t *>(S.hits + kOneTileCols);
    DrawSink<LEN, T> sink{eps, S, &p, &L, &wk, dinfo, Srow / (double)nsample, key, (int64_t)walker * nsample, o, wl, 0xffffffffu};
    visit_tiles<LEN, T>(p, pl, L, nocc, plan, wk, nchunks, chunk, chunk_len, 0u, &next_tile, sink);
    sink.flush();
    flush_winner_list<LEN, T>(o, wl, &wl_base, p, L, wk);
  }
}


template <int LEN, typename T, bool SAMPLED, bool CACHED = false>
__global__ __launch_bounds__(kBlock) __attribute__((amdgpu_waves_per_eu(8, 8)))
void reduce_onepass_list_kernel(const uint64_t *__restrict__ bra, SDParams p, PlanLayout pl, uint32_t nchunks, uint32_t chunk_len, uint32_t max_tiles,
                                const T *__restrict__ plan, T eps, uint32_t nsample, uint64_t seed, uint32_t P, OnepassOut<T> o) {
  static_assert(CACHED || !SAMPLED, "the re-enumerating form has its own kernel");
  reduce_onepass_list_body<LEN, T, SAMPLED, CACHED>(bra, p, pl, nchunks, chunk_len, max_tiles, plan, eps, nsample, seed, P, o);
}

template <int LEN, typename T, bool SAMPLED = false, bool GTILE = false>
__global__ __launch_bounds__(kBlock) void reduce_onepass_list_flush_kernel(const uint64_t *__restrict__ bra, SDParams p, PlanLayout pl, uint32_t nchunks,
                                                                           uint32_t chunk_len, uint32_t max_tiles, const T *__restrict__ plan, T eps,
                                                                           uint32_t nsample, uint64_t seed, uint32_t P, OnepassOut<T> o) {
  reduce_onepass_list_body<LEN, T, SAMPLED, false, true, GTILE>(bra, p, pl, nchunks, chunk_len, max_tiles, plan, eps, nsample, seed, P, o);
}

template <int LEN, typename T, bool GTILE = false>
__global__ __launch_bounds__(kBlock) void reduce_onepass_list_redraw_kernel(const uint64_t *__restrict__ bra, SDParams p, PlanLayout pl, uint32_t nchunks,
                                                                            uint32_t chunk_len, uint32_t max_tiles, const T *__restrict__ plan, T eps,
                                                                            uint32_t nsample, uint64_t seed, uint32_t P, OnepassOut<T> o) {
  reduce_onepass_list_body<LEN, T, true, false, false, GTILE>(bra, p, pl, nchunks, chunk_len, max_tiles, plan, eps, nsample, seed, P, o);
}

template <typename T, bool CPLX>
__global__ __launch_bounds__(kBlock) void reduce_contract_kernel(int64_t nbatch, uint32_t nchunks, uint32_t fixed, uint32_t cap_d,
                                                                 uint32_t nsample, const int32_t *__restrict__ rec_col,
                                                                 const T *__restrict__ rec_w, const int32_t *__restrict__ rec_link,
                                                                 const int32_t *__restrict__ seg_count, const int32_t *__restrict__ srec_col,
                                                                 const T *__restrict__ srec_w, const int32_t *__restrict__ srec_link,
                                                                 const int32_t *__restrict__ dedup_i32, int slot_i32, int row_off, uint32_t ucap,
                                                                 const double *__restrict__ psi_u, const double *__restrict__ psi_t, int divide,
                                                                 double *__restrict__ eloc, double *__restrict__ psi_x) {
  const int lane = threadIdx.x & 63;
  const int64_t walker = (int64_t)blockIdx.x * (kBlock / 64) + (threadIdx.x >> 6);
  if (walker >= nbatch) return;
  double ar = 0.0, ai = 0.0, xr = 0.0, xi = 0.0;
  bool bad = false;
  auto amp = [&](int32_t link, double &re, double &im) {
    const double *src;
    int64_t at;
    if (link >= kDirectLink) {
      src = psi_u; at = link - kDirectLink;
      if ((uint32_t)at >= ucap) { bad = true; re = im = 0.0; return; }
    } else if (link >= 0) {
      if (!dedup_i32) { bad = true; re = im = 0.0; return; }
      const int32_t row = dedup_i32[(int64_t)link * slot_i32 + row_off];
      if (row < 0 || (uint32_t)row >= ucap) { bad = true; re = im = 0.0; return; }
      src = psi_u; at = row;
    } else if (link <= -2) {
      src = psi_t; at = -2 - (int64_t)link;
    } else { bad = true; re = im = 0.0; return; }
    if constexpr (CPLX) { re = src[2 * at]; im = src[2 * at + 1]; }
    else { re = src[at]; im = 0.0; }
  };
  auto visit = [&](int32_t col, double w, int32_t link) {
    if (col < 0) return;
    double re, im;
    amp(link, re, im);
    ar += w * re; ai += w * im;
    if (col == 0) { xr = re; xi = im; }
  };
  const int64_t stride = (int64_t)fixed + cap_d;
  for (uint32_t c = 0; c < nchunks; ++c) {
    const int64_t seg = walker * nchunks + c, base = seg * stride;
    const uint32_t kept = (uint32_t)seg_count[seg];
    if (kept > cap_d) bad = true;
    const uint32_t nslots = fixed + min(kept, cap_d);
    for (uint32_t i = lane; i < nslots; i += 64) visit(rec_col[base + i], (double)rec_w[base + i], rec_link[base + i]);
  }
  for (uint32_t i = lane; i < nsample; i += 64) {
    const int64_t at = walker * nsample + i;
    visit(srec_col[at], (double)srec_w[at], srec_link[at]);
  }
#pragma unroll
  for (int d = 32; d > 0; d >>= 1) {
    ar += __shfl_xor(ar, d); ai += __shfl_xor(ai, d);
    xr += __shfl_xor(xr, d); xi += __shfl_xor(xi, d);
  }
  const bool anybad = __ballot(bad) != 0;
  if (lane == 0) {
    if (anybad) { ar = ai = __builtin_nan(""); }
    if constexpr (CPLX) {
      if (divide) scaled_cdiv(ar, ai, xr, xi, ar, ai);
      eloc[2 * walker] = ar;
      eloc[2 * walker + 1] = ai;
      psi_x[2 * walker] = xr; psi_x[2 * walker + 1] = xi;
    } else {
      eloc[walker] = divide ? ar / xr : ar;
      psi_x[walker] = xr;
    }
  }
}

__global__ __launch_bounds__(kBlock) void reduce_clear_kernel(uint4 *__restrict__ table, size_t n16, uint32_t *__restrict__ counters) {
  const uint4 ones = make_uint4(0xffffffffu, 0xffffffffu, 0xffffffffu, 0xffffffffu);
  for (size_t i = (size_t)blockIdx.x * kBlock + threadIdx.x; i < n16; i += (size_t)gridDim.x * kBlock) table[i] = ones;
  if (blockIdx.x == 0 && threadIdx.x < 4) counters[threadIdx.x] = 0u;
}

}

using namespace pynqs;

static int onepass_geometry(int64_t nbatch, const SDParams &p, bool sampled, uint32_t *nchunks, uint32_t *chunk_len, uint32_t *max_tiles,
                            uint32_t *fixed) {
  const uint32_t ncomb = p.nsd + 1;
  if (sampled) {
    *nchunks = 1;
    *chunk_len = (ncomb + 255u) & ~255u;
  } else {
    plan_chunks(nbatch, ncomb, nchunks, chunk_len);
  }
  *max_tiles = max_tiles_per_chunk(p, *nchunks, *chunk_len);
  const uint32_t tS_all = (p.d1 + kSinglesPerTile - 1) / kSinglesPerTile;
  *fixed = kFixedHead + ((tS_all + *nchunks - 1) / *nchunks) * kSinglesPerTile;
  return 0;
}

static size_t onepass_static_lds(int) { return 16 + (kBlock / 64) * 4 + (kBlock / 64 + 1) * 12 + 64; }

extern "C" int pynqs_reduce_onepass_geometry(int64_t nbatch, int sorb, int nele, int noA, int noB, int eps_sample, int64_t *out4) {
  SDParams p;
  PlanLayout pl;
  if (!out4) return set_error(PYNQS_EINVAL, "null pointer");
  if (!make_sd_params(sorb, nele, noA, noB, &p) || !make_plan_layout(sorb, &pl)) return set_error(PYNQS_EINVAL, "bad sorb/noA/noB (even sorb in [2, 192])");
  if (nbatch < 0 || nbatch > 0x7fffffffll || eps_sample < 0 || eps_sample > 65535) return set_error(PYNQS_EINVAL, "bad nbatch / eps_sample (at most 65535 draws)");
  uint32_t nchunks, chunk_len, max_tiles, fixed;
  onepass_geometry(nbatch, p, eps_sample > 0, &nchunks, &chunk_len, &max_tiles, &fixed);
  const int len = (sorb - 1) / 64 + 1;
  const int64_t slots = out4[2];
  out4[0] = nbatch * (int64_t)nchunks;
  out4[1] = fixed;
  out4[2] = slots > 0 ? slots * dedup_slot_words(len) * 8 : 0;
  const bool lookback = onepass_lds(p, 8, max_tiles, eps_sample > 0, winner_list_cap(eps_sample)) + onepass_static_lds(len) <= 160 * 1024;
  const bool flushing = eps_sample > 0 && p.nsd + 1 > 65536 &&
                        onepass_list_lds(p, 8, max_tiles, true, 2048, (uint32_t)eps_sample, false, true) + 256 + onepass_static_lds(len) <= 160 * 1024;
  out4[3] = lookback || flushing ? 1 : 0;
  return PYNQS_OK;
}

constexpr uint32_t kLongRow = 65536;
struct OnepassForm {
  uint32_t P;
  bool use_list, use_cache, use_flush, use_gtile;
  size_t lds;
  bool use_split = false;
  bool use_row32 = false;
};
static OnepassForm onepass_form(const SDParams &p, size_t esz, uint32_t max_tiles, uint32_t fixed, uint64_t cap_doubles, int eps_sample,
                                bool have_cache, uint32_t chunk_len, bool no_table, bool have_tile_scratch = false, bool have_row_f32 = false) {
  static const int list_env = getenv("PYNQS_OP_LIST") ? atoi(getenv("PYNQS_OP_LIST")) : -1;
  static const int cache_env = getenv("PYNQS_OP_CACHE") ? atoi(getenv("PYNQS_OP_CACHE")) : -1;
  static const int flush_env = getenv("PYNQS_OP_FLUSH") ? atoi(getenv("PYNQS_OP_FLUSH")) : -1;
  const bool sampled = eps_sample > 0;
  const uint64_t seg_cap = (uint64_t)fixed + cap_doubles;
  OnepassForm f;
  f.P = 64;
  while (f.P < seg_cap && f.P < (1u << 20)) f.P <<= 1;
  const bool want_cache = sampled && have_cache && cache_env != 0;
  const bool gtile = sampled && !want_cache && have_tile_scratch;
  const size_t lds_list = onepass_list_lds(p, esz, max_tiles, sampled, f.P, (uint32_t)eps_sample, want_cache, gtile);
  const bool list_fits = seg_cap <= 2048 && lds_list + 256 <= 160 * 1024;
  f.use_list = list_env == 0 ? false : (list_fits && (list_env == 1 || seg_cap <= 1024 || p.nsd + 1 > kLongRow));
  f.use_cache = want_cache && f.use_list;
  f.use_gtile = gtile && f.use_list;
  f.lds = f.use_list ? lds_list : onepass_lds(p, esz, max_tiles, sampled, winner_list_cap(eps_sample));
  static const int split_env = getenv("PYNQS_OP_SPLIT") ? atoi(getenv("PYNQS_OP_SPLIT")) : -1;
  if (sampled && have_row_f32 && split_env != 0 && list_env != 0 && seg_cap <= 1024 && reduce_draw_supported(p, eps_sample)) {
    const uint32_t slots = ((uint32_t)seg_cap + 1u) & ~1u;
    const size_t lds_a = onepass_list_lds(p, esz, max_tiles, true, slots, (uint32_t)eps_sample, false, false, true);
    if (lds_a + 256 <= 160 * 1024) {
      f.P = slots;
      f.use_list = true; f.use_split = true; f.use_cache = f.use_gtile = f.use_flush = false; f.lds = lds_a;
      return f;
    }
  }
  const bool gtile_f = sampled && have_tile_scratch;
  const uint32_t flush_P = flush_list_slots((p.sorb - 1) / 64 + 1, sampled);
  const size_t lds_flush = onepass_list_lds(p, esz, max_tiles, sampled, flush_P, (uint32_t)eps_sample, false, gtile_f);
  const bool long_row = p.nsd + 1 > kLongRow;
  f.use_flush = !f.use_list && flush_env != 0 && lds_flush + 256 <= 160 * 1024 &&
                (long_row || flush_env == 1 || no_table || cap_doubles * 10 <= (uint64_t)chunk_len);
  if (f.use_flush) { f.use_gtile = gtile_f; f.use_cache = false; }
  if (f.use_flush) { f.P = flush_P; f.lds = lds_flush; }
  static const int row32_env = getenv("PYNQS_OP_ROW32") ? atoi(getenv("PYNQS_OP_ROW32")) : -1;
  const bool from_list = f.use_list && !f.use_cache && flush_env != 0;
  if ((f.use_flush || from_list) && sampled && have_row_f32 && row32_env != 0 && row32_fits(esz, flush_P, (uint32_t)eps_sample, gtile_f)) {
    const size_t lds_r = onepass_list_lds(p, esz, max_tiles, true, flush_P, (uint32_t)eps_sample, false, gtile_f, false, true);
    const size_t wg_old = (size_t)160 * 1024 / ((f.use_flush ? lds_flush : f.lds) + 512), wg_new = (size_t)160 * 1024 / (lds_r + 512);
    if (lds_r + 256 <= 160 * 1024 && (row32_env == 1 || wg_new > wg_old || (uint64_t)eps_sample * 8 >= max_tiles)) {
      f.use_row32 = true; f.use_flush = true; f.use_list = false; f.use_cache = false; f.use_gtile = gtile_f; f.P = flush_P; f.lds = lds_r;
    }
  }
  return f;
}

extern "C" int64_t pynqs_reduce_onepass_tile_scratch_bytes(int64_t nbatch, int sorb, int nele, int noA, int noB, int eps_sample) {
  SDParams p;
  PlanLayout pl;
  if (!make_sd_params(sorb, nele, noA, noB, &p) || !make_plan_layout(sorb, &pl) || nbatch < 0 || nbatch > 0x7fffffffll || eps_sample < 0 || eps_sample > 65535) {
    set_error(PYNQS_EINVAL, "bad arguments");
    return -1;
  }
  if (eps_sample == 0) return 0;
  uint32_t nchunks, chunk_len, max_tiles, fixed;
  onepass_geometry(nbatch, p, true, &nchunks, &chunk_len, &max_tiles, &fixed);
  return (int64_t)((size_t)nbatch * tile_scratch_stride(max_tiles));
}

extern "C" int pynqs_reduce_onepass_list_capacity(int64_t nbatch, int sorb, int nele, int noA, int noB, int dtype, int eps_sample,
                                                  int with_row_cache, int without_table, int64_t *cap_doubles) {
  SDParams p;
  PlanLayout pl;
  if (!cap_doubles) return set_error(PYNQS_EINVAL, "null pointer");
  if (!make_sd_params(sorb, nele, noA, noB, &p) || !make_plan_layout(sorb, &pl)) return set_error(PYNQS_EINVAL, "bad sorb/noA/noB (even sorb in [2, 192])");
  if (nbatch < 0 || nbatch > 0x7fffffffll || eps_sample < 0 || eps_sample > 65535 || (dtype != PYNQS_F32 && dtype != PYNQS_F64))
    return set_error(PYNQS_EINVAL, "bad nbatch / eps_sample / dtype");
  uint32_t nchunks, chunk_len, max_tiles, fixed;
  onepass_geometry(nbatch, p, eps_sample > 0, &nchunks, &chunk_len, &max_tiles, &fixed);
  const size_t esz = dtype == PYNQS_F64 ? 8 : 4;
  auto listed = [&](uint64_t cap) {
    const OnepassForm f = onepass_form(p, esz, max_tiles, fixed, cap, eps_sample, with_row_cache != 0, chunk_len, without_table != 0,
                                       eps_sample > 0 && with_row_cache == 0);
    return (f.use_list || f.use_flush) && f.lds + onepass_static_lds(0) <= 160 * 1024;
  };
  *cap_doubles = -1;
  if (listed((uint64_t)1 << 29)) { *cap_doubles = ((int64_t)1 << 30) - 1; return PYNQS_OK; }
  for (uint32_t seg = 2048; seg >= 128; seg >>= 1) {
    if (seg < fixed) break;
    if (listed(seg - fixed)) { *cap_doubles = (int64_t)(seg - fixed); break; }
  }
  if ((int64_t)(chunk_len / 10) > *cap_doubles && listed(chunk_len / 10)) *cap_doubles = chunk_len / 10;
  return PYNQS_OK;
}

extern "C" int pynqs_reduce_onepass_wants_row_f32(int64_t nbatch, int sorb, int nele, int noA, int noB, int dtype, int eps_sample, int64_t cap_doubles,
                                                  int with_tile_scratch, int without_table) {
  SDParams p;
  PlanLayout pl;
  if (!make_sd_params(sorb, nele, noA, noB, &p) || !make_plan_layout(sorb, &pl) || nbatch < 0 || nbatch > 0x7fffffffll || eps_sample < 0 ||
      eps_sample > 65535 || cap_doubles < 0 || (dtype != PYNQS_F32 && dtype != PYNQS_F64)) {
    set_error(PYNQS_EINVAL, "bad arguments");
    return -1;
  }
  if (eps_sample == 0) return 0;
  uint32_t nchunks, chunk_len, max_tiles, fixed;
  onepass_geometry(nbatch, p, true, &nchunks, &chunk_len, &max_tiles, &fixed);
  const size_t esz = dtype == PYNQS_F64 ? 8 : 4;
  const OnepassForm f = onepass_form(p, esz, max_tiles, fixed, (uint64_t)cap_doubles, eps_sample, false, chunk_len, without_table != 0, false, true);
  if (f.use_split) return 1;
  const OnepassForm g = with_tile_scratch ? onepass_form(p, esz, max_tiles, fixed, (uint64_t)cap_doubles, eps_sample, false, chunk_len, without_table != 0, true, true) : f;
  return g.use_row32 ? 2 : 0;
}

extern "C" int64_t pynqs_reduce_onepass_row_f32_elements(int64_t nbatch, int sorb, int nele, int noA, int noB) {
  SDParams p;
  if (!make_sd_params(sorb, nele, noA, noB, &p) || nbatch < 0 || nbatch > 0x7fffffffll) {
    set_error(PYNQS_EINVAL, "bad arguments");
    return -1;
  }
  return (int64_t)((size_t)nbatch * draw_row_stride(p.nsd + 1));
}

extern "C" int pynqs_reduce_onepass(const uint64_t *bra, int64_t nbatch, int sorb, int nele, int noA, int noB, const void *plan, int dtype,
                                    double eps, int eps_sample, uint64_t seed, const pynqs_reduce_io *io, void *stream) {
  pynqs::DeviceScope device_scope_(bra);
  SDParams p;
  PlanLayout pl;
  if (!make_sd_params(sorb, nele, noA, noB, &p) || !make_plan_layout(sorb, &pl)) return set_error(PYNQS_EINVAL, "bad sorb/noA/noB (even sorb in [2, 192])");
  if (nbatch < 0 || nbatch > 0x7fffffffll || (dtype != PYNQS_F32 && dtype != PYNQS_F64)) return set_error(PYNQS_EINVAL, "bad nbatch/dtype");
  if (eps_sample < 0 || eps_sample > 65535) return set_error(PYNQS_EINVAL, "eps_sample must be in [0, 65535]");
  if (!io) return set_error(PYNQS_EINVAL, "null pointer");
  const bool sampled = eps_sample > 0;
  if (!io->counters || !io->uniq_onv || !io->rec_col || !io->rec_w || !io->rec_link || !io->seg_count ||
      (sampled && (!io->srec_col || !io->srec_w || !io->srec_link)))
    return set_error(PYNQS_EINVAL, "null pointer");
  if (io->cap_unique < 1 || io->cap_unique >= (1ll << 30) || io->cap_doubles < 0 || io->cap_doubles >= (1ll << 30) ||
      (io->dedup_table && (io->dedup_slots < 64 || (io->dedup_slots & (io->dedup_slots - 1)) || io->dedup_slots > (1ll << 30) ||
                           2 * io->cap_unique > io->dedup_slots)))
    return set_error(PYNQS_EINVAL, "bad capacities (dedup_slots: power of two >= 2 * cap_unique)");
  if (io->pm1_dtype != PYNQS_F32 && io->pm1_dtype != PYNQS_F64) return set_error(PYNQS_EINVAL, "bad pm1_dtype");
  if (io->lut_table && io->lut_nkeys < 0) return set_error(PYNQS_EINVAL, "bad lut_nkeys");
  hipStream_t st = (hipStream_t)stream;
  const int len = (sorb - 1) / 64 + 1;
  static const bool clear_kernel = !(getenv("PYNQS_REDUCE_CLEAR_KERNEL") && atoi(getenv("PYNQS_REDUCE_CLEAR_KERNEL")) == 0);
  const size_t table_bytes = io->dedup_table ? (size_t)io->dedup_slots * dedup_slot_words(len) * 8 : 0;
  if (clear_kernel && table_bytes && table_bytes % 16 == 0 && ((uintptr_t)io->dedup_table & 15) == 0 && ((uintptr_t)io->counters & 3) == 0) {
    const size_t n16 = table_bytes / 16;
    size_t blocks = (n16 + (size_t)kBlock * 8 - 1) / ((size_t)kBlock * 8);
    if (blocks > 2048) blocks = 2048;
    hipLaunchKernelGGL(reduce_clear_kernel, dim3((uint32_t)blocks), dim3(kBlock), 0, st, (uint4 *)io->dedup_table, n16, (uint32_t *)io->counters);
  } else {
    if (hipMemsetAsync(io->counters, 0, 16, st) != hipSuccess) return check_launch("memset");
    if (table_bytes && hipMemsetAsync(io->dedup_table, 0xFF, table_bytes, st) != hipSuccess) return check_launch("memset");
  }
  if (nbatch == 0) return PYNQS_OK;
  if (!bra || !plan) return set_error(PYNQS_EINVAL, "null pointer");
  uint32_t nchunks, chunk_len, max_tiles, fixed;
  onepass_geometry(nbatch, p, sampled, &nchunks, &chunk_len, &max_tiles, &fixed);
  const uint64_t grid = (uint64_t)nbatch * nchunks;
  if (grid > 0x7fffffffull) return set_error(PYNQS_EINVAL, "grid too large");
  if (grid * ((uint64_t)fixed + (uint64_t)io->cap_doubles) > 0x7fffffffull * 16ull) return set_error(PYNQS_EINVAL, "record arrays too large");
  const size_t esz = dtype == PYNQS_F64 ? 8 : 4;
  const bool have_tiles = io->tile_scratch != nullptr && io->tile_scratch_bytes >= (int64_t)((size_t)nbatch * tile_scratch_stride(max_tiles));
  const OnepassForm form = onepass_form(p, esz, max_tiles, fixed, (uint64_t)io->cap_doubles, eps_sample, io->row_cache != nullptr, chunk_len,
                                        io->dedup_table == nullptr, have_tiles, io->row_f32 != nullptr);
  const uint32_t P = form.P;
  const bool use_list = form.use_list || form.use_flush, use_cache = form.use_cache, use_flush = form.use_flush, use_gtile = form.use_gtile;
  const bool use_split = form.use_split, use_row32 = form.use_row32;
  const size_t lds = form.lds;
  if (lds + onepass_static_lds(len) > 160 * 1024) return set_error(PYNQS_EINVAL, "row too long for the fused form (LDS): use the multi-pass entry points");
  if (!io->dedup_table && !use_list)
    return set_error(PYNQS_EINVAL, "no de-duplication table: only the LIST forms run without one (cap_doubles <= pynqs_reduce_onepass_list_capacity)");
  static const bool verbose = getenv("PYNQS_OP_VERBOSE") != nullptr;
  if (verbose)
    fprintf(stderr, "pynqs_reduce_onepass: %s form%s, LDS %zu bytes per workgroup (walker tables %zu, max_tiles %u, list P %u), %u chunk(s) per walker\n",
            use_split ? "LIST + float32 row copy + sorted draws" : use_row32 ? (use_gtile ? "flushing LIST + float32 row copy (tile sums in global memory)" : "flushing LIST + float32 row copy") : use_flush ? "flushing LIST" : use_list ? (use_gtile ? "LIST (tile sums in global memory)" : "LIST") : "look-back", use_cache ? " with row cache" : "", lds, (size_t)lds_fixed_bytes(p), max_tiles, P, nchunks);
  const double eps_eff = (sampled && !(eps > 0.0)) ? __builtin_inf() : eps;
  if (use_split) return launch_reduce_rowout(bra, nbatch, p, pl, chunk_len, max_tiles, plan, dtype, eps_eff, eps_sample, seed, P, lds, io, fixed, st);
  if (use_row32) return launch_reduce_flush_row32(bra, nbatch, p, pl, chunk_len, max_tiles, plan, dtype, eps_eff, eps_sample, seed, P, lds, io, fixed, use_gtile, st);
#define PYNQS_OP_LAUNCH(TT, SM)                                                                                                      \
  do {                                                                                                                               \
    auto kfn = use_flush ? (use_gtile ? reduce_onepass_list_flush_kernel<LEN, TT, SM, SM> : reduce_onepass_list_flush_kernel<LEN, TT, SM, false>) \
             : use_list ? (use_cache ? reduce_onepass_list_kernel<LEN, TT, SM, SM>                                                   \
                                     : (SM ? (use_gtile ? reduce_onepass_list_redraw_kernel<LEN, TT, true> : reduce_onepass_list_redraw_kernel<LEN, TT, false>) \
                                           : reduce_onepass_list_kernel<LEN, TT, false, false>)) \
                        : reduce_onepass_kernel<LEN, TT, SM>;                                                                        \
    if (lds > 64 * 1024 && hipFuncSetAttribute(reinterpret_cast<const void *>(kfn), hipFuncAttributeMaxDynamicSharedMemorySize,      \
                                               (int)lds) != hipSuccess)                                                              \
      return check_launch("hipFuncSetAttribute");                                                                                   \
    hipLaunchKernelGGL(kfn, dim3((uint32_t)grid), dim3(kBlock), lds, st, bra, p, pl, nchunks, chunk_len, max_tiles, (const TT *)plan, \
                       (TT)eps_eff, (uint32_t)eps_sample, seed, use_list ? P : winner_list_cap(eps_sample), make_out<TT>(io, len, fixed, use_gtile ? max_tiles : 0u));                \
  } while (0)
  DISPATCH_LEN(len, {
    if (dtype == PYNQS_F64) { if (sampled) PYNQS_OP_LAUNCH(double, true); else PYNQS_OP_LAUNCH(double, false); }
    else { if (sampled) PYNQS_OP_LAUNCH(float, true); else PYNQS_OP_LAUNCH(float, false); }
  });
#undef PYNQS_OP_LAUNCH
  return check_launch("reduce_onepass");
}

extern "C" int pynqs_reduce_contract(int64_t nbatch, int sorb, int nele, int noA, int noB, int dtype, int eps_sample,
                                     const pynqs_reduce_io *io, const double *psi_unique, const double *psi_table, int psi_is_complex,
                                     int divide, double *eloc, double *psi_x, void *stream) {
  pynqs::DeviceScope device_scope_(eloc);
  SDParams p;
  if (!make_sd_params(sorb, nele, noA, noB, &p)) return set_error(PYNQS_EINVAL, "bad sorb/noA/noB");
  if (nbatch < 0 || nbatch > 0x7fffffffll || (dtype != PYNQS_F32 && dtype != PYNQS_F64) || eps_sample < 0 || eps_sample > 65535)
    return set_error(PYNQS_EINVAL, "bad nbatch/dtype/eps_sample");
  if (nbatch == 0) return PYNQS_OK;
  if (!io || !io->rec_col || !io->rec_w || !io->rec_link || !io->seg_count || !psi_unique || !eloc || !psi_x ||
      (eps_sample > 0 && (!io->srec_col || !io->srec_w || !io->srec_link)) || (io->lut_table && !psi_table))
    return set_error(PYNQS_EINVAL, "null pointer");
  uint32_t nchunks, chunk_len, max_tiles, fixed;
  onepass_geometry(nbatch, p, eps_sample > 0, &nchunks, &chunk_len, &max_tiles, &fixed);
  const int len = (sorb - 1) / 64 + 1;
  hipStream_t st = (hipStream_t)stream;
  const uint32_t grid = (uint32_t)((nbatch + kBlock / 64 - 1) / (kBlock / 64));
#define PYNQS_CT_LAUNCH(TT, CX)                                                                                                          \
  hipLaunchKernelGGL((reduce_contract_kernel<TT, CX>), dim3(grid), dim3(kBlock), 0, st, nbatch, nchunks, fixed, (uint32_t)io->cap_doubles, \
                     (uint32_t)eps_sample, io->rec_col, (const TT *)io->rec_w, io->rec_link, io->seg_count, io->srec_col,                \
                     (const TT *)io->srec_w, io->srec_link, (const int32_t *)io->dedup_table, dedup_slot_words(len) * 2,                 \
                     dedup_row_offset(len), (uint32_t)io->cap_unique, psi_unique, psi_table, divide, eloc, psi_x)
  if (dtype == PYNQS_F64) { if (psi_is_complex) PYNQS_CT_LAUNCH(double, true); else PYNQS_CT_LAUNCH(double, false); }
  else { if (psi_is_complex) PYNQS_CT_LAUNCH(float, true); else PYNQS_CT_LAUNCH(float, false); }
#undef PYNQS_CT_LAUNCH
  return check_launch("reduce_contract");
}

#ifdef PYNQS_OP_STAMPS
extern "C" int pynqs_debug_stamps(unsigned long long *out) {
  return (int)hipMemcpyFromSymbol(out, HIP_SYMBOL(pynqs::g_stamps), sizeof(unsigned long long) * 8192 * 16);
}
#endif
```

pynqs_amd/grad.py:

```python
from __future__ import annotations

import contextlib
from typing import Union

import torch
from torch import Tensor, nn

from .distributed import all_reduce_packed, get_world_size
from .public_function import split_batch_idx


def grad(nqs: nn.Module, states: Tensor, state_prob: Tensor, eloc: Tensor, e_total: Union[complex, float, Tensor],
         extra_psi_pow: Union[Tensor, float] = 1.0, dtype=torch.double, AD_MAX_DIM: int = -1, empty_shard_state: "Tensor | None" = None) -> Tensor:
    device = states.device
    dim = states.size(0)
    loss_sum = torch.zeros(1, device=device, dtype=torch.double)
    batch = dim if (AD_MAX_DIM == -1 or AD_MAX_DIM > dim) else AD_MAX_DIM
    ends = split_batch_idx(dim, batch) if dim > 0 else []

    def batch_loss_backward(begin: int, end: int) -> None:
        nonlocal loss_sum
        state = states[begin:end]
        if state.is_floating_point():
            state = state.requires_grad_()
        log_psi = nqs(state).to(dtype).log()
        if torch.any(torch.isnan(log_psi)):
            raise ValueError("There are negative numbers in the log-psi, please use complex128")
        prob_b = state_prob[begin:end].real.to(dtype)
        eloc_b = eloc[begin:end].to(dtype)
        c = 1.0 if isinstance(extra_psi_pow, float) else extra_psi_pow[begin:end].to(dtype)
        loss = 2 * (log_psi.conj() * (eloc_b - e_total * c) * prob_b).sum().real
        loss.backward()
        loss_sum += loss.detach()

    no_sync = nqs.no_sync if hasattr(nqs, "no_sync") else contextlib.nullcontext
    begin = 0
    with no_sync():
        for end in ends[:-1]:
            batch_loss_backward(begin, end)
            begin = end
    if ends:
        batch_loss_backward(begin, ends[-1])
    elif get_world_size() > 1 and hasattr(nqs, "no_sync"):
        dummy = empty_shard_state if empty_shard_state is not None else states.new_zeros((1,) + tuple(states.shape[1:]))
        out = nqs(dummy.reshape((1,) + tuple(states.shape[1:])).to(states.dtype)).to(dtype).sum()
        if not bool(torch.isfinite(torch.view_as_real(out) if out.is_complex() else out).all()):
            raise ValueError("empty shard: the ansatz is not finite on the dummy configuration; pass empty_shard_state=<a valid state>")
        (out.real * 0.0).backward()
    return all_reduce_packed([loss_sum], get_world_size())[0]


class GraphedGrad:

    def __init__(self, nqs: nn.Module, n: int, sorb: int, dtype=torch.double, device=None, use_pow: bool = False, warmup: int = 3,
                 check_nan: "bool | None" = None) -> None:
        m = getattr(nqs, "module", nqs)
        self.module, self.dtype = m, dtype
        self.check_nan = (not dtype.is_complex) if check_nan is None else check_nan
        self.params = [p for p in m.parameters() if p.requires_grad]
        self.ptrs = [p.data_ptr() for p in self.params]
        dev = device if device is not None else self.params[0].device
        rdt = dtype.to_real() if dtype.is_complex else dtype
        self.states = torch.zeros((n, sorb), dtype=rdt, device=dev)
        self.prob = torch.zeros(n, dtype=rdt, device=dev)
        self.eloc = torch.zeros(n, dtype=dtype, device=dev)
        self.e_total = torch.zeros((), dtype=dtype, device=dev)
        self.pow = torch.ones(n, dtype=dtype, device=dev) if use_pow else None
        self.flat = torch.zeros(sum(p.numel() for p in self.params), dtype=self.params[0].dtype, device=dev)
        assert all(p.dtype == self.flat.dtype for p in self.params), "one parameter dtype per module"
        views, o = [], 0
        for p in self.params:
            views.append(self.flat[o:o + p.numel()].view_as(p))
            o += p.numel()
        self.views = views
        self.loss = torch.zeros(1, dtype=torch.double, device=dev)
        self.events = None
        self.graph = torch.cuda.CUDAGraph()
        side = torch.cuda.Stream(device=dev)
        side.wait_stream(torch.cuda.current_stream(dev))
        with torch.cuda.stream(side):
            for _ in range(warmup):
                self._body()
        torch.cuda.current_stream(dev).wait_stream(side)
        with torch.cuda.graph(self.graph, capture_error_mode="thread_local"):
            self._body()

    def _body(self) -> None:
        log_psi = self.module(self.states).to(self.dtype).log()
        c = 1.0 if self.pow is None else self.pow
        loss = 2 * (log_psi.conj() * (self.eloc - self.e_total * c) * self.prob).sum().real
        grads = torch.autograd.grad(loss, self.params)
        for v, g in zip(self.views, grads):
            v.copy_(g)
        self.loss.copy_(loss.detach().reshape(1))

    def _check_params(self) -> None:
        cur = [p for p in self.module.parameters() if p.requires_grad]
        if len(cur) != len(self.params) or any(a is not b or a.data_ptr() != ptr for a, b, ptr in zip(cur, self.params, self.ptrs)):
            raise RuntimeError("GraphedGrad: the module's parameters were replaced or re-allocated since the graph was captured (the replay "
                               "would read the old storage and fill the old tensors' .grad); build a new GraphedGrad")

    def __call__(self, states: Tensor, state_prob: Tensor, eloc: Tensor, e_total, extra_psi_pow=1.0) -> Tensor:
        self._check_params()
        self.states.copy_(states)
        self.prob.copy_(state_prob.real if state_prob.is_complex() else state_prob)
        self.eloc.copy_(eloc)
        self.e_total.copy_((e_total if isinstance(e_total, Tensor) else torch.as_tensor(e_total)).reshape(()))
        if self.pow is not None:
            self.pow.copy_(extra_psi_pow)
        self.graph.replay()
        if self.check_nan and bool(torch.isnan(self.loss).any()):
            for p in self.params:
                p.grad = None
            raise ValueError("There are negative numbers in the log-psi, please use complex128")
        ws = get_world_size()
        ev = None
        if self.events is not None:
            ev = [torch.cuda.Event(enable_timing=True) for _ in range(2)]
            ev[0].record()
        if ws > 1:
            import torch.distributed as dist

            dist.all_reduce(self.flat, dist.ReduceOp.SUM)
            self.flat.div_(ws)
        if ev is not None:
            ev[1].record()
            self.events.append(ev)
        for p, v in zip(self.params, self.views):
            p.grad = v
        return all_reduce_packed([self.loss], ws)[0]


class FusedRbmGrad:

    def __init__(self, nqs: nn.Module, sorb: int) -> None:
        from . import _native as N
        from .rbm import ComplexRBM, RealRBM

        m = getattr(nqs, "module", nqs)
        if isinstance(m, ComplexRBM):
            self.flavour, self.names = N.RBM_COMPLEX, ("params_weights", "params_hidden_bias", "params_visible_bias")
        elif isinstance(m, RealRBM) and getattr(m, "rbm_type", "real") == "real":
            self.flavour, self.names = N.RBM_REAL, ("weights", "hidden_bias", "visible_bias")
        else:
            raise ValueError("FusedRbmGrad: the module is not a real (rbm_type 'real') or complex-parameter RBM")
        self.N, self.module, self.sorb = N, m, sorb
        params = [getattr(m, nm) for nm in self.names]
        if any(p.dtype != torch.float64 or not p.is_cuda for p in params):
            raise ValueError("FusedRbmGrad: float64 parameters on the GPU")
        dev = params[0].device
        self.H = params[0].size(0)
        self.shapes = [p.shape for p in params]
        self.flat = torch.zeros(sum(p.numel() for p in params) + 1, dtype=torch.float64, device=dev)
        self.views, o = [], 0
        for p in params:
            self.views.append(self.flat[o:o + p.numel()].view_as(p))
            o += p.numel()
        self.loss = self.flat[o:o + 1]
        self.work = None
        self.events = None

    @property
    def params(self):
        ps = [getattr(self.module, nm) for nm in self.names]
        if any(p.dtype != torch.float64 or p.device != self.flat.device for p in ps):
            raise ValueError("FusedRbmGrad: float64 parameters on the GPU")
        if [p.shape for p in ps] != self.shapes:
            raise ValueError(f"FusedRbmGrad: parameter shapes changed since construction ({self.shapes} -> {[p.shape for p in ps]})")
        return ps

    def __call__(self, onv: Tensor, state_prob: Tensor, eloc: Tensor, e_total, extra_psi_pow=1.0) -> Tensor:
        N, dev = self.N, self.flat.device
        n = onv.size(0)
        if onv.dtype != torch.uint8 or onv.dim() != 2 or onv.size(1) != 8 * ((self.sorb - 1) // 64 + 1) or onv.device != dev:
            raise ValueError("FusedRbmGrad: walkers as packed onv uint8[n, 8 len] on the parameters' device")
        cplx = eloc.is_complex()
        prob = (state_prob.real if state_prob.is_complex() else state_prob).to(torch.float64).contiguous()
        el = eloc.to(torch.complex128 if cplx else torch.float64).contiguous()
        et = (e_total if isinstance(e_total, Tensor) else torch.as_tensor(e_total)).to(device=dev, dtype=el.dtype).reshape(1).contiguous()
        pw = None
        if isinstance(extra_psi_pow, Tensor):
            if extra_psi_pow.is_complex():
                raise ValueError("FusedRbmGrad: extra_psi_pow must be real")
            pw = extra_psi_pow.to(torch.float64).contiguous()
        elif float(extra_psi_pow) != 1.0:
            pw = torch.full((n,), float(extra_psi_pow), dtype=torch.float64, device=dev)
        need = N.lib().pynqs_rbm_grad_workspace(n, self.sorb, self.H, self.flavour)
        if self.work is None or self.work.numel() * 8 < need:
            self.work = torch.empty(max(need // 8, 1), dtype=torch.float64, device=dev)
        params = self.params
        W, hb, vb = (p.detach().contiguous() for p in params)
        gw, ghb, gvb = self.views
        ws = get_world_size()
        loss_out = torch.empty(1, dtype=torch.float64, device=dev) if ws == 1 else None
        N.check(N.lib().pynqs_rbm_grad_loss(onv.contiguous().data_ptr(), n, self.sorb, W.data_ptr(), hb.data_ptr(), vb.data_ptr(), self.H,
                                            self.flavour, prob.data_ptr(), el.data_ptr(), int(cplx), et.data_ptr(),
                                            pw.data_ptr() if pw is not None else None, gw.data_ptr(), ghb.data_ptr(), gvb.data_ptr(),
                                            self.loss.data_ptr(), loss_out.data_ptr() if loss_out is not None else None, self.work.data_ptr(),
                                            torch.cuda.current_stream(dev).cuda_stream), "pynqs_rbm_grad_loss")
        ev = None
        if self.events is not None:
            ev = [torch.cuda.Event(enable_timing=True) for _ in range(2)]
            ev[0].record()
        if ws > 1:
            import torch.distributed as dist

            dist.all_reduce(self.flat, dist.ReduceOp.SUM)
            self.flat.div_(ws)
        if ev is not None:
            ev[1].record()
            self.events.append(ev)
        for p, v in zip(params, self.views):
            p.grad = v
        return self.loss * ws if ws > 1 else loss_out


class FusedJastrowRbmGrad:

    names = ("weights", "hidden_bias", "visible_bias", "jastrow")

    def __init__(self, nqs: nn.Module, sorb: int) -> None:
        from . import _native as N
        from .rbm import JastrowRBM

        m = getattr(nqs, "module", nqs)
        if not isinstance(m, JastrowRBM):
            raise ValueError("FusedJastrowRbmGrad: the module is not a pynqs_amd.rbm.JastrowRBM")
        self.N, self.module, self.sorb = N, m, sorb
        params = [getattr(m, nm) for nm in self.names]
        if any(p.dtype != torch.float64 or not p.is_cuda for p in params):
            raise ValueError("FusedJastrowRbmGrad: float64 parameters on the GPU")
        if params[0].size(1) != sorb:
            raise ValueError(f"FusedJastrowRbmGrad: the module has {params[0].size(1)} orbitals, not {sorb}")
        dev = params[0].device
        self.H = params[0].size(0)
        self.shapes = [p.shape for p in params]
        self.flat = torch.zeros(sum(p.numel() for p in params) + 1, dtype=torch.float64, device=dev)
        self.views, o = [], 0
        for p in params:
            self.views.append(self.flat[o:o + p.numel()].view_as(p))
            o += p.numel()
        self.loss = self.flat[o:o + 1]
        self.loss_jastrow = torch.zeros(1, dtype=torch.float64, device=dev)
        self.work = None
        self.events = None

    @property
    def params(self):
        ps = [getattr(self.module, nm) for nm in self.names]
        if any(p.dtype != torch.float64 or p.device != self.flat.device for p in ps):
            raise ValueError("FusedJastrowRbmGrad: float64 parameters on the GPU")
        if [p.shape for p in ps] != self.shapes:
            raise ValueError(f"FusedJastrowRbmGrad: parameter shapes changed since construction ({self.shapes} -> {[p.shape for p in ps]})")
        return ps

    def __call__(self, onv: Tensor, state_prob: Tensor, eloc: Tensor, e_total, extra_psi_pow=1.0) -> Tensor:
        N, dev = self.N, self.flat.device
        n = onv.size(0)
        if onv.dtype != torch.uint8 or onv.dim() != 2 or onv.size(1) != 8 * ((self.sorb - 1) // 64 + 1) or onv.device != dev:
            raise ValueError("FusedJastrowRbmGrad: walkers as packed onv uint8[n, 8 len] on the parameters' device")
        if eloc.is_complex():
            raise ValueError("FusedJastrowRbmGrad: the amplitude is real: a real local energy")
        prob = (state_prob.real if state_prob.is_complex() else state_prob).to(torch.float64).contiguous()
        el = eloc.to(torch.float64).contiguous()
        et = (e_total if isinstance(e_total, Tensor) else torch.as_tensor(e_total)).to(device=dev, dtype=torch.float64).reshape(1).contiguous()
        pw = None
        if isinstance(extra_psi_pow, Tensor):
            if extra_psi_pow.is_complex():
                raise ValueError("FusedJastrowRbmGrad: extra_psi_pow must be real")
            pw = extra_psi_pow.to(torch.float64).contiguous()
        elif float(extra_psi_pow) != 1.0:
            pw = torch.full((n,), float(extra_psi_pow), dtype=torch.float64, device=dev)
        lib = N.lib()
        need = max(lib.pynqs_rbm_grad_workspace(n, self.sorb, self.H, N.RBM_REAL), lib.pynqs_jastrow_grad_workspace(n, self.sorb))
        if self.work is None or self.work.numel() * 8 < need:
            self.work = torch.empty(max(need // 8, 1), dtype=torch.float64, device=dev)
        params = self.params
        W, hb, vb, M = (p.detach().contiguous() for p in params)
        gw, ghb, gvb, gm = self.views
        x = onv.contiguous()
        st = torch.cuda.current_stream(dev).cuda_stream
        pwp = pw.data_ptr() if pw is not None else None
        N.check(lib.pynqs_rbm_grad(x.data_ptr(), n, self.sorb, W.data_ptr(), hb.data_ptr(), vb.data_ptr(), self.H, N.RBM_REAL, prob.data_ptr(),
                                   el.data_ptr(), 0, et.data_ptr(), pwp, gw.data_ptr(), ghb.data_ptr(), gvb.data_ptr(), self.loss.data_ptr(),
                                   self.work.data_ptr(), st), "pynqs_rbm_grad")
        N.check(lib.pynqs_jastrow_grad(x.data_ptr(), n, self.sorb, M.data_ptr(), prob.data_ptr(), el.data_ptr(), et.data_ptr(), pwp, gm.data_ptr(),
                                       self.loss_jastrow.data_ptr(), self.work.data_ptr(), st), "pynqs_jastrow_grad")
        self.loss += self.loss_jastrow
        ws = get_world_size()
        ev = None
        if self.events is not None:
            ev = [torch.cuda.Event(enable_timing=True) for _ in range(2)]
            ev[0].record()
        if ws > 1:
            import torch.distributed as dist

            dist.all_reduce(self.flat, dist.ReduceOp.SUM)
            self.flat.div_(ws)
        if ev is not None:
            ev[1].record()
            self.events.append(ev)
        for p, v in zip(params, self.views):
            p.grad = v
        return self.loss * ws if ws > 1 else self.loss.clone()
```

pynqs_amd/reduce_front.py:

```python
from __future__ import annotations

import ctypes as C
import os
from typing import Optional, Tuple

import torch
from torch import Tensor

from . import _native as N

OVERFLOW_DOUBLES, OVERFLOW_TABLE, OVERFLOW_UNIQUE = 1, 2, 4
ROW_CACHE = True
ROW_CACHE_MAX_BYTES = 8 << 30
ROW_F32 = os.environ.get("PYNQS_ROW_F32", "1") != "0"
ROW_F32_MAX_BYTES = int(os.environ.get("PYNQS_ROW_F32_MAX_BYTES", str(16 << 30)))
TILE_SCRATCH_MIN_ROW = int(os.environ.get("PYNQS_TILE_SCRATCH_MIN_ROW", "65536"))


def _pow2_at_least(v: int) -> int:
    c = 64
    while c < v:
        c <<= 1
    return c


def geometry(n: int, sorb: int, nele: int, noa: int, nob: int, eps_sample: int, dedup_slots: int = 0) -> Tuple[int, int, int, bool]:
    out = (C.c_int64 * 4)(0, 0, dedup_slots, 0)
    N.check(N.lib().pynqs_reduce_onepass_geometry(n, sorb, nele, noa, nob, int(eps_sample), out), "pynqs_reduce_onepass_geometry")
    return int(out[0]), int(out[1]), int(out[2]), bool(out[3])


def supported(n: int, sorb: int, nele: int, noa: int, nob: int, eps_sample: int) -> bool:
    if sorb % 2 or not 0 <= eps_sample <= 65535:
        return False
    try:
        return geometry(n, sorb, nele, noa, nob, eps_sample)[3]
    except RuntimeError:
        return False


def wants_row_cache(n: int, ncomb: int, eps_sample: int, nchunks: int, esz: int) -> bool:
    return bool(eps_sample > 0 and nchunks == 1 and ROW_CACHE and eps_sample * 64 >= ncomb and n * ncomb * esz <= ROW_CACHE_MAX_BYTES)


def list_capacity(n: int, sorb: int, nele: int, noa: int, nob: int, eps_sample: int, h_dtype: torch.dtype = torch.float64,
                  without_table: bool = False) -> int:
    ncomb = int(N.lib().pynqs_num_sd(sorb, noa, nob)) + 1
    esz = 8 if h_dtype == torch.float64 else 4
    nseg = geometry(n, sorb, nele, noa, nob, eps_sample)[0]
    cache = wants_row_cache(n, ncomb, int(eps_sample), nseg // max(n, 1) if n else 1, esz)
    out = C.c_int64(-1)
    N.check(N.lib().pynqs_reduce_onepass_list_capacity(n, sorb, nele, noa, nob, N.PYNQS_F64 if esz == 8 else N.PYNQS_F32, int(eps_sample),
                                                       int(cache), int(without_table), C.byref(out)), "pynqs_reduce_onepass_list_capacity")
    return int(out.value)


class ReduceFrontEnd:

    def __init__(self, n: int, sorb: int, nele: int, noa: int, nob: int, eps_sample: int, h_dtype: torch.dtype, device,
                 cap_doubles: int, cap_unique: int, pm1_dtype: torch.dtype = torch.float64, keep_onv: bool = True, want_pm1: bool = True,
                 dedup: bool = True) -> None:
        if h_dtype not in (torch.float64, torch.float32) or pm1_dtype not in (torch.float64, torch.float32):
            raise TypeError("float32 / float64 only")
        self.n, self.sorb, self.nele, self.noa, self.nob = int(n), sorb, nele, noa, nob
        self.eps_sample = int(eps_sample)
        self.h_dtype, self.pm1_dtype, self.device = h_dtype, pm1_dtype, torch.device(device)
        self.L = (sorb - 1) // 64 + 1
        self.cap_doubles, self.cap_unique = max(int(cap_doubles), 0), max(int(cap_unique), 1)
        self.dedup_slots = _pow2_at_least(2 * self.cap_unique)
        self.nseg, self.fixed, table_bytes, ok = geometry(self.n, sorb, nele, noa, nob, self.eps_sample, self.dedup_slots)
        if not ok:
            raise RuntimeError("row too long for the fused REDUCE front end (LDS): use reduce_compact / reduce_compact_sampled")
        self.nchunks = self.nseg // max(self.n, 1) if self.n else 1
        self.stride = self.fixed + self.cap_doubles
        dev, L = self.device, self.L
        slots = max(self.nseg * self.stride, 1)
        self.rec_col = torch.empty(slots, dtype=torch.int32, device=dev)
        self.rec_w = torch.zeros(slots, dtype=h_dtype, device=dev)
        self.rec_onv = torch.zeros((slots, 8 * L), dtype=torch.uint8, device=dev) if keep_onv else None
        self.rec_link = torch.empty(slots, dtype=torch.int32, device=dev)
        self.seg_count = torch.zeros(max(self.nseg, 1), dtype=torch.int32, device=dev)
        ns = max(self.n * self.eps_sample, 1)
        self.srec_col = torch.empty(ns, dtype=torch.int32, device=dev)
        self.srec_w = torch.zeros(ns, dtype=h_dtype, device=dev)
        self.srec_onv = torch.zeros((ns, 8 * L), dtype=torch.uint8, device=dev) if keep_onv else None
        self.srec_link = torch.empty(ns, dtype=torch.int32, device=dev)
        self.row_sum = torch.zeros(max(self.n, 1), dtype=torch.float64, device=dev)
        self.dedup = bool(dedup)
        self.table = torch.empty(table_bytes // 4, dtype=torch.int32, device=dev) if self.dedup else None
        self.slot_i32 = table_bytes // 4 // self.dedup_slots
        self.row_off = 2 if L == 1 else 1
        self.uniq_onv = torch.zeros((self.cap_unique, 8 * L), dtype=torch.uint8, device=dev)
        self.uniq_pm1 = torch.ones((self.cap_unique, sorb), dtype=pm1_dtype, device=dev) if want_pm1 else None
        self.uniq_parent = torch.zeros(self.cap_unique, dtype=torch.int32, device=dev)
        self.counters = torch.zeros(4, dtype=torch.int32, device=dev)
        self.seed_dev = torch.zeros(1, dtype=torch.int64, device=dev)
        ncomb = int(N.lib().pynqs_num_sd(sorb, noa, nob)) + 1
        esz = 8 if h_dtype == torch.float64 else 4
        self.row_cache = None
        self.row_f32, self.row_f32_form = None, 0
        if self.eps_sample > 0 and ROW_F32:
            self.row_f32_form = int(N.lib().pynqs_reduce_onepass_wants_row_f32(
                self.n, sorb, nele, noa, nob, N.PYNQS_F64 if esz == 8 else N.PYNQS_F32, self.eps_sample, self.cap_doubles,
                int(ncomb > TILE_SCRATCH_MIN_ROW), int(not self.dedup)))
            if self.row_f32_form in (1, 2):
                nel = int(N.lib().pynqs_reduce_onepass_row_f32_elements(self.n, sorb, nele, noa, nob))
                if self.row_f32_form == 1 or 4 * nel <= ROW_F32_MAX_BYTES:
                    self.row_f32 = torch.empty(max(nel, 1), dtype=torch.float32, device=dev)
        if self.row_f32 is None and wants_row_cache(self.n, ncomb, self.eps_sample, self.nchunks, esz):
            self.row_cache = torch.empty(max(self.n * ncomb, 1), dtype=h_dtype, device=dev)
        self.tile_scratch = None
        if self.eps_sample > 0 and self.row_cache is None and (self.row_f32 is None or self.row_f32_form == 2) and ncomb > TILE_SCRATCH_MIN_ROW:
            nb = int(N.lib().pynqs_reduce_onepass_tile_scratch_bytes(self.n, sorb, nele, noa, nob, self.eps_sample))
            if nb > 0:
                self.tile_scratch = torch.empty(nb, dtype=torch.uint8, device=dev)
        self._lut = None
        self._io = self._make_io()

    def _make_io(self, rec_w: Optional[Tensor] = None, srec_w: Optional[Tensor] = None, lut=None) -> N.ReduceIO:
        io = N.ReduceIO()
        io.cap_doubles, io.cap_unique, io.dedup_slots = self.cap_doubles, self.cap_unique, self.dedup_slots
        io.rec_col, io.rec_w = self.rec_col.data_ptr(), (self.rec_w if rec_w is None else rec_w).data_ptr()
        io.rec_onv = self.rec_onv.data_ptr() if self.rec_onv is not None else None
        io.rec_link, io.seg_count = self.rec_link.data_ptr(), self.seg_count.data_ptr()
        io.srec_col, io.srec_w = self.srec_col.data_ptr(), (self.srec_w if srec_w is None else srec_w).data_ptr()
        io.srec_onv = self.srec_onv.data_ptr() if self.srec_onv is not None else None
        io.srec_link, io.row_sum = self.srec_link.data_ptr(), self.row_sum.data_ptr()
        io.dedup_table, io.uniq_onv = (self.table.data_ptr() if self.table is not None else None), self.uniq_onv.data_ptr()
        io.uniq_pm1 = self.uniq_pm1.data_ptr() if self.uniq_pm1 is not None else None
        io.pm1_dtype = N.PYNQS_F64 if self.pm1_dtype == torch.float64 else N.PYNQS_F32
        io.lut_is_hash = 1
        io.lut_table = lut.table.data_ptr() if lut is not None else None
        io.lut_nkeys = lut.nkeys if lut is not None else 0
        io.counters = self.counters.data_ptr()
        io.seed_dev = self.seed_dev.data_ptr()
        io.row_cache = self.row_cache.data_ptr() if self.row_cache is not None else None
        io.uniq_parent = self.uniq_parent.data_ptr()
        io.tile_scratch = self.tile_scratch.data_ptr() if self.tile_scratch is not None else None
        io.tile_scratch_bytes = self.tile_scratch.numel() if self.tile_scratch is not None else 0
        io.row_f32 = self.row_f32.data_ptr() if self.row_f32 is not None else None
        return io

    def record_stream(self, stream) -> None:
        for t in vars(self).values():
            if isinstance(t, Tensor) and t.is_cuda:
                t.record_stream(stream)

    def run(self, x: Tensor, plan: Tensor, eps: float, seed: int = 0, lut=None) -> None:
        if x.size(0) != self.n or not x.is_cuda or x.dtype != torch.uint8 or not x.is_contiguous():
            raise RuntimeError("x must be a contiguous uint8 CUDA tensor with the front end's number of walkers")
        code = N.PYNQS_F64 if self.h_dtype == torch.float64 else N.PYNQS_F32
        if lut is not self._lut:
            self._lut, self._io = lut, self._make_io(lut=lut)
        st = torch.cuda.current_stream(self.device).cuda_stream
        N.check(N.lib().pynqs_reduce_onepass(x.data_ptr(), self.n, self.sorb, self.nele, self.noa, self.nob, plan.data_ptr(), code,
                                             float(eps), self.eps_sample, int(seed) & (2**64 - 1), C.byref(self._io), st),
                "pynqs_reduce_onepass")

    def contract(self, values_unique: Tensor, values_table: Optional[Tensor] = None, divide: bool = True,
                 rec_w: Optional[Tensor] = None, srec_w: Optional[Tensor] = None) -> Tuple[Tensor, Tensor]:
        cplx = values_unique.is_complex()
        vt = torch.complex128 if cplx else torch.float64
        vu = values_unique.to(vt).contiguous()
        tb = values_table.to(vt).contiguous() if values_table is not None else None
        if self._lut is not None and tb is None:
            raise RuntimeError("the records refer to a wave-function table: pass its values")
        io = self._io if rec_w is None and srec_w is None else self._make_io(rec_w, srec_w, self._lut)
        out = torch.empty(self.n, dtype=vt, device=self.device)
        ax = torch.empty(self.n, dtype=vt, device=self.device)
        code = N.PYNQS_F64 if (rec_w if rec_w is not None else self.rec_w).dtype == torch.float64 else N.PYNQS_F32
        st = torch.cuda.current_stream(self.device).cuda_stream
        N.check(N.lib().pynqs_reduce_contract(self.n, self.sorb, self.nele, self.noa, self.nob, code, self.eps_sample, C.byref(io),
                                              vu.data_ptr(), tb.data_ptr() if tb is not None else None, int(cplx), int(divide),
                                              out.data_ptr(), ax.data_ptr(), st), "pynqs_reduce_contract")
        return out, ax

    def counters_host(self) -> Tuple[int, int, int]:
        c = self.counters.tolist()
        return int(c[0]), int(c[1]), int(c[2])

    def overflowed(self, counters: Optional[Tuple[int, int, int]] = None) -> bool:
        nu, flags, mx = counters if counters is not None else self.counters_host()
        return bool(flags) or nu > self.cap_unique or mx > self.cap_doubles

    def table_rows(self) -> Tensor:
        return self.table.view(self.dedup_slots, self.slot_i32)[:, self.row_off]

    def rows_of(self, link: Tensor) -> Tensor:
        link = link.long()
        direct = link >= (1 << 30)
        rows = torch.where(direct, link - (1 << 30), torch.zeros_like(link))
        if not bool(direct.all()):
            rows = torch.where(direct, rows, self.table_rows().long()[torch.where(direct, torch.zeros_like(link), link)])
        return rows

    def count_records(self) -> int:
        col = self.rec_col.view(self.nseg, self.stride)
        slot = torch.arange(self.stride, device=self.device).unsqueeze(0)
        kept = self.seg_count[: self.nseg].clamp(max=self.cap_doubles).unsqueeze(1)
        m = int(torch.where(slot < self.fixed, col >= 0, slot < self.fixed + kept).sum())
        if self.eps_sample > 0:
            m += int((self.srec_col[: self.n * self.eps_sample] >= 0).sum())
        return m

    def records(self):
        dev = self.device
        col = self.rec_col.view(self.nseg, self.stride)
        slot = torch.arange(self.stride, device=dev).unsqueeze(0)
        kept = self.seg_count[: self.nseg].clamp(max=self.cap_doubles).unsqueeze(1)
        valid = torch.where(slot < self.fixed, col >= 0, slot < self.fixed + kept).reshape(-1)
        idx = torch.nonzero(valid).squeeze(1)
        walker = (idx // self.stride) // self.nchunks
        parts = [(walker, self.rec_col[idx], self.rec_w[idx], self.rec_link[idx], self.rec_onv[idx] if self.rec_onv is not None else None)]
        if self.eps_sample > 0:
            sidx = torch.nonzero(self.srec_col[: self.n * self.eps_sample] >= 0).squeeze(1)
            parts.append((sidx // self.eps_sample, self.srec_col[sidx], self.srec_w[sidx], self.srec_link[sidx],
                          self.srec_onv[sidx] if self.srec_onv is not None else None))
        cat = lambda k: torch.cat([p[k] for p in parts])
        drawn = torch.cat([torch.zeros(p[0].numel(), dtype=torch.bool, device=dev) if i == 0 else torch.ones(p[0].numel(), dtype=torch.bool, device=dev)
                           for i, p in enumerate(parts)])
        return cat(0), cat(1), cat(2), cat(3), (cat(4) if self.rec_onv is not None else None), drawn


class ReduceStep:

    def __init__(self, front: ReduceFrontEnd, plan: Tensor, eps: float, amplitude, lut=None, lut_values: Optional[Tensor] = None,
                 seed: int = 0, graph: bool = False) -> None:
        self.front, self.plan, self.eps, self.amplitude = front, plan, float(eps), amplitude
        self.lut, self.lut_values, self.seed = lut, lut_values, int(seed)
        self.x = torch.zeros((front.n, 8 * front.L), dtype=torch.uint8, device=front.device)
        self.eloc = self.psi_x = None
        self._graph = None
        self._want_graph = graph

    def _body(self) -> None:
        fe = self.front
        fe.run(self.x, self.plan, self.eps, self.seed, self.lut)
        if fe.eps_sample:
            fe.seed_dev.add_(1)
        with torch.no_grad():
            psi_u = self.amplitude(fe.uniq_pm1)
        self.eloc, self.psi_x = fe.contract(psi_u, self.lut_values)

    def __call__(self, x: Tensor) -> Tuple[Tensor, Tensor]:
        self.x.copy_(x)
        if not self._want_graph:
            self._body()
        elif self._graph is None:
            s = torch.cuda.Stream(self.front.device)
            s.wait_stream(torch.cuda.current_stream(self.front.device))
            with torch.cuda.stream(s):
                for _ in range(2):
                    self._body()
            torch.cuda.current_stream(self.front.device).wait_stream(s)
            g = torch.cuda.CUDAGraph()
            with torch.cuda.graph(g):
                self._body()
            self._graph = g
            g.replay()
        else:
            self._graph.replay()
        return self.eloc, self.psi_x

    def check(self) -> Tuple[int, int, int]:
        cnt = self.front.counters_host()
        if self.front.overflowed(cnt):
            raise OverflowError(f"REDUCE front end too small: needed {cnt[0]} distinct rows (capacity {self.front.cap_unique}), "
                                f"{cnt[2]} kept columns in a segment (capacity {self.front.cap_doubles}), flags {cnt[1]}")
        return cnt
```

Before: 10.04 million.

## Add single-workgroup moments, one-pass RBM gradient and batched contract kernels

Adds three alternative kernel forms. The first is a single-workgroup weighted-moments reduction used automatically for small n, which avoids the multi-block reduction and its completion counter. The second is a one-pass RBM gradient kernel that can stage weights in LDS. The third is a batched reduce-contract kernel, now the default, which processes several records per step so their loads can overlap. Each is exposed through new *_form entry points, and the serial and two-pass paths stay available for comparison at the cost of more code and more template instantiations.

New measurement: 10.25 million, median of 6. +2.1%, better.

```diff
diff --git a/include/pynqs_amd.h b/include/pynqs_amd.h
--- a/include/pynqs_amd.h
+++ b/include/pynqs_amd.h
@@ -159,6 +159,12 @@
 int pynqs_weighted_moments(const double *x, int is_complex, const double *prob, int64_t n, void *workspace, void *stream);
 int pynqs_weighted_moments_finish(const double *x, int is_complex, const double *prob, int64_t n, void *workspace, double inv_world,
                                   double counts, double *out5, void *stream);
+#define PYNQS_MOMENTS_AUTO 0
+#define PYNQS_MOMENTS_BLOCKS 1
+#define PYNQS_MOMENTS_ONEGROUP 2
+int64_t pynqs_moments_onegroup_max(void);
+int pynqs_weighted_moments_form(const double *x, int is_complex, const double *prob, int64_t n, void *workspace, double inv_world,
+                                double counts, double *out5, int form, void *stream);
 
 int64_t pynqs_reduce_tiles(int64_t nbatch, int sorb, int nele, int noA, int noB);
 int pynqs_reduce_count(const uint64_t *bra, int64_t nbatch, int sorb, int nele, int noA, int noB,
@@ -217,6 +223,11 @@
 int pynqs_reduce_contract(int64_t nbatch, int sorb, int nele, int noA, int noB, int dtype, int eps_sample,
                           const pynqs_reduce_io *io, const double *psi_unique, const double *psi_table, int psi_is_complex,
                           int divide, double *eloc, double *psi_x, void *stream);
+#define PYNQS_CONTRACT_BATCHED 0
+#define PYNQS_CONTRACT_SERIAL 1
+int pynqs_reduce_contract_form(int64_t nbatch, int sorb, int nele, int noA, int noB, int dtype, int eps_sample,
+                               const pynqs_reduce_io *io, const double *psi_unique, const double *psi_table, int psi_is_complex,
+                               int divide, double *eloc, double *psi_x, int form, void *stream);
 
 #define PYNQS_RBM_COMPLEX 4
 int pynqs_rbm_forward(const uint64_t *onv, int64_t n, int sorb, const double *weights, const double *hidden_bias,
@@ -248,6 +259,13 @@
                         int eloc_is_complex, const double *e_total, const double *pow, double *grad_weights,
                         double *grad_hidden_bias, double *grad_visible_bias, double *loss, double *loss_copy, void *workspace,
                         void *stream);
+#define PYNQS_GRAD_ONEPASS 0
+#define PYNQS_GRAD_TWOPASS 1
+int pynqs_rbm_grad_loss_form(const uint64_t *onv, int64_t n, int sorb, const double *weights, const double *hidden_bias,
+                             const double *visible_bias, int nhidden, int flavour, const double *prob, const double *eloc,
+                             int eloc_is_complex, const double *e_total, const double *pow, double *grad_weights,
+                             double *grad_hidden_bias, double *grad_visible_bias, double *loss, double *loss_copy, void *workspace,
+                             int schedule, int block, void *stream);
 
 #define PYNQS_SR_RHO 0
 #define PYNQS_SR_RHS2 1
diff --git a/pynqs_amd/_native.py b/pynqs_amd/_native.py
--- a/pynqs_amd/_native.py
+++ b/pynqs_amd/_native.py
@@ -66,6 +66,8 @@
     "pynqs_stats_finish": (_int, [_vp, _dbl, _dbl, _vp, _vp]),
     "pynqs_weighted_moments": (_int, [_vp, _int, _vp, _i64, _vp, _vp]),
     "pynqs_weighted_moments_finish": (_int, [_vp, _int, _vp, _i64, _vp, _dbl, _dbl, _vp, _vp]),
+    "pynqs_moments_onegroup_max": (_i64, []),
+    "pynqs_weighted_moments_form": (_int, [_vp, _int, _vp, _i64, _vp, _dbl, _dbl, _vp, _int, _vp]),
     "pynqs_reduce_tiles": (_i64, [_i64, _int, _int, _int, _int]),
     "pynqs_reduce_count": (_int, [_vp, _i64, _int, _int, _int, _int, _vp, _int, _dbl, _vp, _vp]),
     "pynqs_reduce_count_sums": (_int, [_vp, _i64, _int, _int, _int, _int, _vp, _int, _dbl, _vp, _vp, _vp]),
@@ -101,7 +103,10 @@
     "pynqs_rbm_grad_workspace": (_i64, [_i64, _int, _int, _int]),
     "pynqs_rbm_grad": (_int, [_vp, _i64, _int, _vp, _vp, _vp, _int, _int, _vp, _vp, _int, _vp, _vp, _vp, _vp, _vp, _vp, _vp, _vp]),
     "pynqs_rbm_grad_loss": (_int, [_vp, _i64, _int, _vp, _vp, _vp, _int, _int, _vp, _vp, _int, _vp, _vp, _vp, _vp, _vp, _vp, _vp, _vp, _vp]),
-    "pynqs_reduce_contract": (_int, [_i64, _int, _int, _int, _int, _int, _int, C.POINTER(ReduceIO), _vp, _vp, _int, _int, _vp, _vp, _vp]),    "pynqs_mcmc_rbm_supported": (_int, [_int, _int, _int]),
+    "pynqs_rbm_grad_loss_form": (_int, [_vp, _i64, _int, _vp, _vp, _vp, _int, _int, _vp, _vp, _int, _vp, _vp, _vp, _vp, _vp, _vp, _vp, _vp, _int, _int, _vp]),
+    "pynqs_reduce_contract": (_int, [_i64, _int, _int, _int, _int, _int, _int, C.POINTER(ReduceIO), _vp, _vp, _int, _int, _vp, _vp, _vp]),
+    "pynqs_reduce_contract_form": (_int, [_i64, _int, _int, _int, _int, _int, _int, C.POINTER(ReduceIO), _vp, _vp, _int, _int, _vp, _vp, _int, _vp]),
+    "pynqs_mcmc_rbm_supported": (_int, [_int, _int, _int]),
     "pynqs_mcmc_rbm": (_int, [_vp, _i64, _int, _int, _int, _vp, _int, _int, C.c_uint64, C.c_uint64, C.c_uint64, _int, _int, _vp, _vp, _vp, _vp]),
     "pynqs_rbm_sr_workspace": (_i64, [_i64, _int, _int, _int]),
     "pynqs_rbm_sr_prepare": (_int, [_vp, _i64, _int, _vp, _vp, _int, _int, _vp, _vp, _vp, _vp]),
diff --git a/pynqs_amd/csrc/kernels_gfmc.hip b/pynqs_amd/csrc/kernels_gfmc.hip
--- a/pynqs_amd/csrc/kernels_gfmc.hip
+++ b/pynqs_amd/csrc/kernels_gfmc.hip
@@ -195,6 +195,79 @@
   }
 }
 
+constexpr int kMomentsGroupThreads = 1024;
+constexpr int kMomentsBatch = 8;
+
+template <bool CPLX, bool FINISH>
+__global__ __launch_bounds__(kMomentsGroupThreads) void moments_onegroup_kernel(const double *__restrict__ x, const double *__restrict__ prob,
+                                                                                int64_t n, int blocks, double *__restrict__ out,
+                                                                                double inv_world, double counts, double *__restrict__ out5) {
+  constexpr int NW = kMomentsGroupThreads / 64, VW = kBlock / 64;
+  __shared__ double wsum[kMomentBlocks * VW][4];
+  __shared__ double part[kMomentBlocks][4];
+  const int tid = threadIdx.x, lane = tid & 63, wave = tid >> 6;
+  const int V = blocks * VW;
+  for (int v0 = 0; v0 < V; v0 += NW * kMomentsBatch) {
+    double a[4 * kMomentsBatch];
+    double pv[kMomentsBatch], rv[kMomentsBatch], iv[kMomentsBatch];
+#pragma unroll
+    for (int sl = 0; sl < kMomentsBatch; ++sl) {
+      const int64_t i = (int64_t)(v0 + wave * kMomentsBatch + sl) * 64 + lane;
+      const bool in = i < n && v0 + wave * kMomentsBatch + sl < V;
+      pv[sl] = in ? prob[i] : 0.0;
+      rv[sl] = in ? (CPLX ? x[2 * i] : x[i]) : 0.0;
+      iv[sl] = CPLX && in ? x[2 * i + 1] : 0.0;
+    }
+#pragma unroll
+    for (int sl = 0; sl < kMomentsBatch; ++sl) {
+      const int64_t i = (int64_t)(v0 + wave * kMomentsBatch + sl) * 64 + lane;
+      double s[4] = {0.0, 0.0, 0.0, 0.0};
+      if (i < n && v0 + wave * kMomentsBatch + sl < V) {
+        const double p = pv[sl];
+        const double re = rv[sl], im = CPLX ? iv[sl] : 0.0;
+        s[0] += p * re; s[1] += p * im; s[2] += p * (re * re + im * im); s[3] += p;
+      }
+#pragma unroll
+      for (int k = 0; k < 4; ++k) a[4 * sl + k] = s[k];
+    }
+#pragma unroll
+    for (int d = 32, m = 4 * kMomentsBatch; m > 1; d >>= 1, m >>= 1) {
+      const bool hi = (lane & d) != 0;
+#pragma unroll
+      for (int j = 0; j < m / 2; ++j) {
+        const double keep = hi ? a[2 * j + 1] : a[2 * j], send = hi ? a[2 * j] : a[2 * j + 1];
+        a[j] = keep + __shfl_xor(send, d);
+      }
+    }
+    static_assert(4 * kMomentsBatch == 32, "five halving steps, then distance 1");
+    a[0] += __shfl_xor(a[0], 1);
+    const int k = ((lane >> 5) & 1) | (((lane >> 4) & 1) << 1);
+    const int sl = ((lane >> 3) & 1) | (((lane >> 2) & 1) << 1) | (((lane >> 1) & 1) << 2);
+    const int v = v0 + wave * kMomentsBatch + sl;
+    if (!(lane & 1) && v < V) wsum[v][k] = a[0];
+  }
+  __syncthreads();
+  if (tid < blocks * 4) {
+    const int b = tid >> 2, k = tid & 3;
+    double t = 0.0;
+#pragma unroll
+    for (int w = 0; w < VW; ++w) t += wsum[b * VW + w][k];
+    out[4 * (1 + b) + k] = t;
+    part[b][k] = t;
+  }
+  __syncthreads();
+  if (tid < 4) {
+    double t = 0.0;
+    for (int b = 0; b < blocks; ++b) t += part[b][tid];
+    out[tid] = t;
+    if constexpr (FINISH) wsum[0][tid] = t;
+  }
+  if constexpr (FINISH) {
+    __syncthreads();
+    if (tid == 0) stats_finish(&wsum[0][0], inv_world, counts, out5);
+  }
+}
+
 __global__ void stats_finish_kernel(const double *__restrict__ m, double inv_world, double counts, double *__restrict__ out) {
   stats_finish(m, inv_world, counts, out);
 }
@@ -210,18 +283,33 @@
 
 extern "C" int64_t pynqs_moments_workspace(void) { return 8 * 4 * (pynqs::kMomentBlocks + 1) + 8; }
 
+constexpr int64_t kMomentsOneGroupMax = (int64_t)kMomentBlocks * kBlock;
+
+extern "C" int64_t pynqs_moments_onegroup_max(void) { return kMomentsOneGroupMax; }
+
 static int weighted_moments_launch(const double *x, int is_complex, const double *prob, int64_t n, void *workspace, bool finish, double inv_world,
-                                   double counts, double *out5, void *stream) {
+                                   double counts, double *out5, int form, void *stream) {
   pynqs::DeviceScope device_scope_(x);
   if (n < 0) return set_error(PYNQS_EINVAL, "bad n");
   if (!workspace || (n > 0 && (!x || !prob))) return set_error(PYNQS_EINVAL, "null pointer");
   if (finish && (!out5 || !(counts > 0.0))) return set_error(PYNQS_EINVAL, "bad arguments");
+  if (form < PYNQS_MOMENTS_AUTO || form > PYNQS_MOMENTS_ONEGROUP || (form == PYNQS_MOMENTS_ONEGROUP && n > (int64_t)kMomentBlocks * kBlock))
+    return set_error(PYNQS_EINVAL, "bad form (the single-workgroup form takes n <= 32768)");
   double *out = (double *)workspace;
   unsigned int *done = (unsigned int *)(out + 4 * (kMomentBlocks + 1));
   int64_t blocks = (n + kBlock - 1) / kBlock;
   if (blocks > kMomentBlocks) blocks = kMomentBlocks;
   if (blocks < 1) blocks = 1;
   hipStream_t st = (hipStream_t)stream;
+  if (form == PYNQS_MOMENTS_ONEGROUP || (form == PYNQS_MOMENTS_AUTO && n <= kMomentsOneGroupMax)) {
+#define PYNQS_MK(C, F)                                                                                                                    \
+  hipLaunchKernelGGL((moments_onegroup_kernel<C, F>), dim3(1), dim3(kMomentsGroupThreads), 0, st, x, prob, n, (int)blocks, out, inv_world, \
+                     counts, out5)
+    if (finish) { if (is_complex) PYNQS_MK(true, true); else PYNQS_MK(false, true); }
+    else { if (is_complex) PYNQS_MK(true, false); else PYNQS_MK(false, false); }
+#undef PYNQS_MK
+    return check_launch("weighted_moments");
+  }
 #define PYNQS_MK(C, F) \
   hipLaunchKernelGGL((moments_kernel<C, F>), dim3((uint32_t)blocks), dim3(kBlock), 0, st, x, prob, n, out, done, inv_world, counts, out5)
   if (finish) { if (is_complex) PYNQS_MK(true, true); else PYNQS_MK(false, true); }
@@ -231,10 +319,15 @@
 }
 
 extern "C" int pynqs_weighted_moments(const double *x, int is_complex, const double *prob, int64_t n, void *workspace, void *stream) {
-  return weighted_moments_launch(x, is_complex, prob, n, workspace, false, 1.0, 1.0, nullptr, stream);
+  return weighted_moments_launch(x, is_complex, prob, n, workspace, false, 1.0, 1.0, nullptr, PYNQS_MOMENTS_AUTO, stream);
 }
 
 extern "C" int pynqs_weighted_moments_finish(const double *x, int is_complex, const double *prob, int64_t n, void *workspace, double inv_world,
                                              double counts, double *out5, void *stream) {
-  return weighted_moments_launch(x, is_complex, prob, n, workspace, true, inv_world, counts, out5, stream);
-}
+  return weighted_moments_launch(x, is_complex, prob, n, workspace, true, inv_world, counts, out5, PYNQS_MOMENTS_AUTO, stream);
+}
+
+extern "C" int pynqs_weighted_moments_form(const double *x, int is_complex, const double *prob, int64_t n, void *workspace, double inv_world,
+                                           double counts, double *out5, int form, void *stream) {
+  return weighted_moments_launch(x, is_complex, prob, n, workspace, out5 != nullptr, inv_world, counts, out5, form, stream);
+}
diff --git a/pynqs_amd/csrc/kernels_rbm_grad.hip b/pynqs_amd/csrc/kernels_rbm_grad.hip
--- a/pynqs_amd/csrc/kernels_rbm_grad.hip
+++ b/pynqs_amd/csrc/kernels_rbm_grad.hip
@@ -1,6 +1,8 @@
 #include "detcore.h"
 #include "launch.h"
 #include "rbm_math.h"
+
+#include <type_traits>
 
 namespace pynqs {
 
@@ -158,6 +160,209 @@
   }
 }
 
+constexpr int kGradSuper = 2 * kGradHidden;
+constexpr int kGradWLds = 28 * 1024;
+
+template <int LEN, bool CPLX, int B, bool WLDS>
+__global__ __launch_bounds__(B) void rbm_grad_onepass_kernel(const uint64_t *__restrict__ onv, int64_t n, int sorb, int H,
+                                                                  const double *__restrict__ W, const double *__restrict__ hb,
+                                                                  const double *__restrict__ vb, const double *__restrict__ prob,
+                                                                  const double *__restrict__ eloc, bool eloc_cplx,
+                                                                  const double *__restrict__ e_total, const double *__restrict__ pw,
+                                                                  double *__restrict__ partial, int64_t stride) {
+  constexpr int C = CPLX ? 2 : 1;
+  __shared__ uint64_t xs[kGradWalkers][LEN];
+  __shared__ double tc[kGradWalkers][kGradSuper + 1][C];
+  __shared__ double cf[kGradWalkers][C];
+  extern __shared__ __align__(16) double wl[];
+  constexpr int NQ = B / kGradWalkers;
+  constexpr int HC = kGradHidden / NQ;
+  constexpr int NA = 2 * HC;
+  const int tid = threadIdx.x, w = tid % kGradWalkers, q = tid / kGradWalkers;
+  const int64_t i = (int64_t)blockIdx.x * kGradWalkers + w;
+  const bool valid = i < n;
+  const int64_t row = valid ? i : n - 1;
+  uint64_t ket[LEN];
+#pragma unroll
+  for (int k = 0; k < LEN; ++k) ket[k] = onv[row * LEN + k];
+  double fr = 0.0, fi = 0.0;
+  if (valid) {
+    const double pr = prob[i], c = pw ? pw[i] : 1.0;
+    const double er = eloc_cplx ? eloc[2 * i] : eloc[i], ei = eloc_cplx ? eloc[2 * i + 1] : 0.0;
+    const double tr = e_total[0], ti = eloc_cplx ? e_total[1] : 0.0;
+    fr = pr * (er - tr * c);
+    fi = pr * (ei - ti * c);
+  }
+  if (q == 0) {
+#pragma unroll
+    for (int k = 0; k < LEN; ++k) xs[w][k] = ket[k];
+    cf[w][0] = fr;
+    if constexpr (CPLX) cf[w][1] = -fi;
+  }
+  double *__restrict__ out = partial + (int64_t)blockIdx.x * stride;
+  double lre = 0.0, lim = 0.0;
+  const int SP = sorb + 1;
+  for (int hs = 0; hs < H; hs += kGradSuper) {
+    const int nrows = min(kGradSuper, H - hs);
+    if constexpr (WLDS) {
+      const double *__restrict__ Wg = W + (size_t)hs * sorb * C;
+      const int cnt = nrows * sorb * C;
+#pragma unroll 8
+      for (int k = tid; k < cnt; k += B) wl[k] = Wg[k];
+      __syncthreads();
+    } else {
+      if (hs) __syncthreads();
+    }
+    double tr[NA], ti[NA];
+    const int hfirst = hs + HC * q;
+    const int np = hfirst + kGradHidden < H ? 2 : hfirst < H ? 1 : 0;
+    auto chain = [&](auto npass, const double *Wp, int r0) {
+      constexpr int N = decltype(npass)::value * HC;
+      std::conditional_t<WLDS, int, size_t> rw[N];
+#pragma unroll
+      for (int a = 0; a < N; ++a) {
+        const int h = min(hs + kGradHidden * (a / HC) + HC * q + (a % HC), H - 1);
+        tr[a] = CPLX ? hb[2 * h] : hb[h];
+        ti[a] = CPLX ? hb[2 * h + 1] : 0.0;
+        rw[a] = (std::conditional_t<WLDS, int, size_t>)(h - r0) * sorb;
+      }
+      constexpr int OU = WLDS ? 2 : 4;
+      int o = 0;
+      for (; o + OU <= sorb; o += OU) {
+        double wr[OU][N], wi[OU][N];
+#pragma unroll
+        for (int u = 0; u < OU; ++u)
+#pragma unroll
+          for (int a = 0; a < N; ++a) {
+            if constexpr (CPLX) { wr[u][a] = Wp[(rw[a] + o + u) * 2]; wi[u][a] = Wp[(rw[a] + o + u) * 2 + 1]; }
+            else { wr[u][a] = Wp[rw[a] + o + u]; wi[u][a] = 0.0; }
+          }
+#pragma unroll
+        for (int u = 0; u < OU; ++u) {
+          const double x = pm1_of<LEN>(ket, o + u);
+#pragma unroll
+          for (int a = 0; a < N; ++a) {
+            tr[a] = fma(x, wr[u][a], tr[a]);
+            if constexpr (CPLX) ti[a] = fma(x, wi[u][a], ti[a]);
+          }
+        }
+      }
+      for (; o < sorb; ++o) {
+        const double x = pm1_of<LEN>(ket, o);
+#pragma unroll
+        for (int a = 0; a < N; ++a) {
+          if constexpr (CPLX) {
+            tr[a] = fma(x, Wp[(rw[a] + o) * 2], tr[a]);
+            ti[a] = fma(x, Wp[(rw[a] + o) * 2 + 1], ti[a]);
+          } else {
+            tr[a] = fma(x, Wp[rw[a] + o], tr[a]);
+          }
+        }
+      }
+    };
+#pragma unroll
+    for (int a = 0; a < NA; ++a) { tr[a] = 0.0; ti[a] = 0.0; }
+    if constexpr (WLDS) {
+      if (np == 2) chain(std::integral_constant<int, 2>{}, wl, hs);
+      else if (np == 1) chain(std::integral_constant<int, 1>{}, wl, hs);
+    } else {
+      if (np == 2) chain(std::integral_constant<int, 2>{}, W, 0);
+      else if (np == 1) chain(std::integral_constant<int, 1>{}, W, 0);
+    }
+#pragma unroll
+    for (int a = 0; a < NA; ++a) {
+      const int hh = kGradHidden * (a / HC) + HC * q + (a % HC);
+      const bool live = hs + hh < H;
+      if (!live) {
+        tc[w][hh][0] = 0.0;
+        if constexpr (CPLX) tc[w][hh][1] = 0.0;
+        continue;
+      }
+      const double ax = fabs(tr[a]), e = exp(-2.0 * ax), s = tr[a] < 0.0 ? -1.0 : 1.0;
+      double yr, yi = 0.0;
+      if constexpr (CPLX) {
+        double sn, cs;
+        sincos_mod(2.0 * ti[a], sn, cs);
+        const double den = fma(2.0 * e, cs, fma(e, e, 1.0));
+        yr = s * (1.0 - e * e) / den;
+        yi = 2.0 * e * sn / den;
+        const double u = fma(e, cs, 1.0), v = -s * e * sn;
+        lre += ax + 0.5 * log(u * u + v * v);
+        lim += s * ti[a] + atan2(v, u);
+        tc[w][hh][0] = yr * fr + yi * fi;
+        tc[w][hh][1] = yi * fr - yr * fi;
+      } else {
+        yr = s * (1.0 - e) / (1.0 + e);
+        lre += ax + log1p(e);
+        tc[w][hh][0] = yr * fr;
+      }
+    }
+    __syncthreads();
+    const int nout = nrows * SP;
+    for (int k = tid; k < nout; k += B) {
+      const int hh = k / SP, o = k - hh * SP;
+      double ar = 0.0, ai = 0.0;
+      if (o < sorb) {
+        const int word = o >> 6, bit = o & 63;
+#pragma unroll 8
+        for (int v = 0; v < kGradWalkers; ++v) {
+          const bool up = (xs[v][word] >> bit) & 1ull;
+          const double a = tc[v][hh][0];
+          ar += up ? a : -a;
+          if constexpr (CPLX) { const double b = tc[v][hh][1]; ai += up ? b : -b; }
+        }
+      } else {
+#pragma unroll 8
+        for (int v = 0; v < kGradWalkers; ++v) {
+          ar += tc[v][hh][0];
+          if constexpr (CPLX) ai += tc[v][hh][1];
+        }
+      }
+      const int64_t at = (int64_t)(hs + hh) * SP + o;
+      out[C * at] = ar;
+      if constexpr (CPLX) out[C * at + 1] = ai;
+    }
+  }
+  const int64_t off_vb = (int64_t)H * SP;
+  for (int o = tid; o < sorb; o += B) {
+    const int word = o >> 6, bit = o & 63;
+    double ar = 0.0, ai = 0.0;
+#pragma unroll 4
+    for (int v = 0; v < kGradWalkers; ++v) {
+      const bool up = (xs[v][word] >> bit) & 1ull;
+      ar += up ? cf[v][0] : -cf[v][0];
+      if constexpr (CPLX) ai += up ? cf[v][1] : -cf[v][1];
+    }
+    out[C * (off_vb + o)] = ar;
+    if constexpr (CPLX) out[C * (off_vb + o) + 1] = ai;
+  }
+  if (vb && q == 0) {
+    for (int o = 0; o < sorb; ++o) {
+      const double x = pm1_of<LEN>(ket, o);
+      lre = fma(x, CPLX ? vb[2 * o] : vb[o], lre);
+      if constexpr (CPLX) lim = fma(x, vb[2 * o + 1], lim);
+    }
+  }
+  __syncthreads();
+  double *lr = &tc[0][0][0];
+  lr[(q * kGradWalkers + w) * 2] = lre;
+  lr[(q * kGradWalkers + w) * 2 + 1] = lim;
+  __syncthreads();
+  if (tid < 64) {
+    double l = 0.0;
+    if (q == 0) {
+      double re = 0.0, im = 0.0;
+#pragma unroll
+      for (int k = 0; k < NQ; ++k) { re += lr[(k * kGradWalkers + w) * 2]; im += lr[(k * kGradWalkers + w) * 2 + 1]; }
+      im -= 6.283185307179586476925 * rint(im * 0.15915494309189533577);
+      l = valid ? 2.0 * (re * fr + im * fi) : 0.0;
+    }
+#pragma unroll
+    for (int d = 32; d > 0; d >>= 1) l += __shfl_xor(l, d);
+    if (tid == 0) out[C * (off_vb + sorb)] = l;
+  }
+}
+
 template <bool CPLX>
 __global__ __launch_bounds__(kBlock) void rbm_grad_reduce_kernel(const double *__restrict__ partial, int64_t stride, int ngroups, int sorb, int H,
                                                                  double *__restrict__ gw, double *__restrict__ ghb, double *__restrict__ gvb,
@@ -231,13 +436,16 @@
   return b == 256 ? 256 : 512;
 }
 
-extern "C" int pynqs_rbm_grad_loss(const uint64_t *onv, int64_t n, int sorb, const double *weights, const double *hidden_bias,
-                                   const double *visible_bias, int nhidden, int flavour, const double *prob, const double *eloc,
-                                   int eloc_is_complex, const double *e_total, const double *pow, double *grad_weights, double *grad_hidden_bias,
-                                   double *grad_visible_bias, double *loss, double *loss_copy, void *workspace, void *stream) {
+extern "C" int pynqs_rbm_grad_loss_form(const uint64_t *onv, int64_t n, int sorb, const double *weights, const double *hidden_bias,
+                                        const double *visible_bias, int nhidden, int flavour, const double *prob, const double *eloc,
+                                        int eloc_is_complex, const double *e_total, const double *pow, double *grad_weights,
+                                        double *grad_hidden_bias, double *grad_visible_bias, double *loss, double *loss_copy, void *workspace,
+                                        int schedule, int block, void *stream) {
   pynqs::DeviceScope device_scope_(onv);
   if (n < 0 || n > 0x7fffffffll * kGradWalkers || sorb < 1 || sorb > kMaxSorb || nhidden < 1) return set_error(PYNQS_EINVAL, "bad n/sorb/nhidden");
   if (flavour != PYNQS_RBM_REAL && flavour != PYNQS_RBM_COMPLEX) return set_error(PYNQS_EINVAL, "rbm_grad: flavour must be PYNQS_RBM_REAL or PYNQS_RBM_COMPLEX");
+  if ((schedule != PYNQS_GRAD_ONEPASS && schedule != PYNQS_GRAD_TWOPASS) || (block != 0 && block != 256 && block != 512))
+    return set_error(PYNQS_EINVAL, "rbm_grad: bad schedule / block");
   if (!weights || !hidden_bias || !grad_weights || !grad_hidden_bias || (n > 0 && (!onv || !prob || !eloc || !e_total || !workspace)))
     return set_error(PYNQS_EINVAL, "null pointer");
   const bool cplx = flavour == PYNQS_RBM_COMPLEX;
@@ -246,15 +454,30 @@
   hipStream_t st = (hipStream_t)stream;
   double *partial = (double *)workspace;
   if (groups > 0) {
-    const bool wide = grad_block() == 512;
+    const bool wide = (block ? block : grad_block()) == 512;
+    if (schedule == PYNQS_GRAD_TWOPASS) {
 #define PYNQS_RG(C, B)                                                                                                                         \
   hipLaunchKernelGGL((rbm_grad_partial_kernel<LEN, C, B>), dim3((uint32_t)groups), dim3(B), 0, st, onv, n, sorb, nhidden, weights, hidden_bias, \
                      visible_bias, prob, eloc, eloc_is_complex != 0, e_total, pow, partial, stride)
-    DISPATCH_LEN(len, {
-      if (cplx) { if (wide) PYNQS_RG(true, 512); else PYNQS_RG(true, 256); }
-      else { if (wide) PYNQS_RG(false, 512); else PYNQS_RG(false, 256); }
-    });
+      DISPATCH_LEN(len, {
+        if (cplx) { if (wide) PYNQS_RG(true, 512); else PYNQS_RG(true, 256); }
+        else { if (wide) PYNQS_RG(false, 512); else PYNQS_RG(false, 256); }
+      });
 #undef PYNQS_RG
+    } else {
+      const size_t wbytes = (size_t)(nhidden < kGradSuper ? nhidden : kGradSuper) * sorb * (cplx ? 16 : 8);
+      const bool wlds = wbytes <= (size_t)kGradWLds;
+#define PYNQS_RG(C, B, L)                                                                                                                    \
+  hipLaunchKernelGGL((rbm_grad_onepass_kernel<LEN, C, B, L>), dim3((uint32_t)groups), dim3(B), L ? wbytes : 0, st, onv, n, sorb, nhidden, weights, \
+                     hidden_bias, visible_bias, prob, eloc, eloc_is_complex != 0, e_total, pow, partial, stride)
+#define PYNQS_RG2(C, B) do { if (wlds) PYNQS_RG(C, B, true); else PYNQS_RG(C, B, false); } while (0)
+      DISPATCH_LEN(len, {
+        if (cplx) { if (wide) PYNQS_RG2(true, 512); else PYNQS_RG2(true, 256); }
+        else { if (wide) PYNQS_RG2(false, 512); else PYNQS_RG2(false, 256); }
+      });
+#undef PYNQS_RG2
+#undef PYNQS_RG
+    }
   }
   const int64_t nout = (int64_t)nhidden * (sorb + 1) + sorb + 1;
   const uint32_t g2 = (uint32_t)((nout + 63) / 64);
@@ -267,6 +490,14 @@
   return check_launch("rbm_grad");
 }
 
+extern "C" int pynqs_rbm_grad_loss(const uint64_t *onv, int64_t n, int sorb, const double *weights, const double *hidden_bias,
+                                   const double *visible_bias, int nhidden, int flavour, const double *prob, const double *eloc,
+                                   int eloc_is_complex, const double *e_total, const double *pow, double *grad_weights, double *grad_hidden_bias,
+                                   double *grad_visible_bias, double *loss, double *loss_copy, void *workspace, void *stream) {
+  return pynqs_rbm_grad_loss_form(onv, n, sorb, weights, hidden_bias, visible_bias, nhidden, flavour, prob, eloc, eloc_is_complex, e_total, pow,
+                                  grad_weights, grad_hidden_bias, grad_visible_bias, loss, loss_copy, workspace, PYNQS_GRAD_ONEPASS, 0, stream);
+}
+
 extern "C" int pynqs_rbm_grad(const uint64_t *onv, int64_t n, int sorb, const double *weights, const double *hidden_bias,
                               const double *visible_bias, int nhidden, int flavour, const double *prob, const double *eloc,
                               int eloc_is_complex, const double *e_total, const double *pow, double *grad_weights, double *grad_hidden_bias,
diff --git a/pynqs_amd/csrc/kernels_reduce_onepass.hip b/pynqs_amd/csrc/kernels_reduce_onepass.hip
--- a/pynqs_amd/csrc/kernels_reduce_onepass.hip
+++ b/pynqs_amd/csrc/kernels_reduce_onepass.hip
@@ -549,6 +549,118 @@
   }
 }
 
+#ifndef PYNQS_CONTRACT_BATCH
+#define PYNQS_CONTRACT_BATCH 8
+#endif
+constexpr int kContractBatch = PYNQS_CONTRACT_BATCH;
+
+__device__ __forceinline__ void contract_add(double &ar, double &ai, double w, double re, double im) {
+  ar = fma(w, re, ar);
+  ai = fma(w, im, ai);
+}
+
+template <typename T, bool CPLX, int U>
+__global__ __launch_bounds__(kBlock) void reduce_contract_batched_kernel(int64_t nbatch, uint32_t nchunks, uint32_t fixed, uint32_t cap_d,
+                                                                         uint32_t nsample, const int32_t *__restrict__ rec_col,
+                                                                         const T *__restrict__ rec_w, const int32_t *__restrict__ rec_link,
+                                                                         const int32_t *__restrict__ seg_count, const int32_t *__restrict__ srec_col,
+                                                                         const T *__restrict__ srec_w, const int32_t *__restrict__ srec_link,
+                                                                         const int32_t *__restrict__ dedup_i32, int slot_i32, int row_off, uint32_t ucap,
+                                                                         const double *__restrict__ psi_u, const double *__restrict__ psi_t, int divide,
+                                                                         double *__restrict__ eloc, double *__restrict__ psi_x) {
+  const uint32_t lane = threadIdx.x & 63;
+  const int64_t walker = (int64_t)blockIdx.x * (kBlock / 64) + (threadIdx.x >> 6);
+  if (walker >= nbatch) return;
+  double ar = 0.0, ai = 0.0, xr = 0.0, xi = 0.0;
+  bool bad = false;
+  auto run = [&](const int32_t *__restrict__ colp, const T *__restrict__ wp, const int32_t *__restrict__ lp, uint32_t count) {
+    int32_t coln[U];
+#pragma unroll
+    for (int u = 0; u < U; ++u) {
+      const uint32_t i = lane + 64u * u;
+      coln[u] = i < count ? colp[i] : -1;
+    }
+    for (uint32_t i0 = lane; i0 < count; i0 += 64u * U) {
+      int32_t col[U], link[U];
+      T w[U];
+#pragma unroll
+      for (int u = 0; u < U; ++u) {
+        col[u] = coln[u];
+        const uint32_t i = i0 + 64u * u;
+        w[u] = col[u] >= 0 ? wp[i] : T(0);
+        link[u] = col[u] >= 0 ? lp[i] : -1;
+      }
+#pragma unroll
+      for (int u = 0; u < U; ++u) {
+        const uint32_t i = i0 + 64u * (U + u);
+        coln[u] = i < count ? colp[i] : -1;
+      }
+      int64_t at[U];
+      bool tab[U];
+#pragma unroll
+      for (int u = 0; u < U; ++u) {
+        const int32_t l = link[u];
+        tab[u] = false;
+        at[u] = -1;
+        if (col[u] >= 0) {
+          if (l >= kDirectLink) at[u] = l - kDirectLink;
+          else if (l >= 0) { if (dedup_i32) at[u] = dedup_i32[(int64_t)l * slot_i32 + row_off]; }
+          else if (l <= -2) { tab[u] = true; at[u] = -2 - (int64_t)l; }
+        }
+      }
+      double re[U], im[U];
+#pragma unroll
+      for (int u = 0; u < U; ++u) {
+        re[u] = 0.0; im[u] = 0.0;
+        if (col[u] >= 0) {
+          if (tab[u]) {
+            if constexpr (CPLX) { re[u] = psi_t[2 * at[u]]; im[u] = psi_t[2 * at[u] + 1]; }
+            else re[u] = psi_t[at[u]];
+          } else if (at[u] >= 0 && (uint64_t)at[u] < (uint64_t)ucap) {
+            if constexpr (CPLX) { re[u] = psi_u[2 * at[u]]; im[u] = psi_u[2 * at[u] + 1]; }
+            else re[u] = psi_u[at[u]];
+          } else {
+            bad = true;
+          }
+        }
+      }
+#pragma unroll
+      for (int u = 0; u < U; ++u) {
+        if (col[u] >= 0) {
+          contract_add(ar, ai, (double)w[u], re[u], im[u]);
+          if (col[u] == 0) { xr = re[u]; xi = im[u]; }
+        }
+      }
+    }
+  };
+  const int64_t stride = (int64_t)fixed + cap_d;
+  for (uint32_t c = 0; c < nchunks; ++c) {
+    const int64_t seg = walker * nchunks + c, base = seg * stride;
+    const uint32_t kept = (uint32_t)seg_count[seg];
+    if (kept > cap_d) bad = true;
+    run(rec_col + base, rec_w + base, rec_link + base, fixed + min(kept, cap_d));
+  }
+  if (nsample) run(srec_col + walker * nsample, srec_w + walker * nsample, srec_link + walker * nsample, nsample);
+#pragma unroll
+  for (int d = 32; d > 0; d >>= 1) {
+    ar += __shfl_xor(ar, d); ai += __shfl_xor(ai, d);
+    xr += __shfl_xor(xr, d); xi += __shfl_xor(xi, d);
+  }
+  const bool anybad = __ballot(bad) != 0;
+  if (lane == 0) {
+    if (anybad) { ar = ai = __builtin_nan(""); }
+    if constexpr (CPLX) {
+      if (divide) scaled_cdiv(ar, ai, xr, xi, ar, ai);
+      eloc[2 * walker] = ar;
+      eloc[2 * walker + 1] = ai;
+      psi_x[2 * walker] = xr; psi_x[2 * walker + 1] = xi;
+    } else {
+      eloc[walker] = divide ? ar / xr : ar;
+      psi_x[walker] = xr;
+    }
+  }
+}
+
 __global__ __launch_bounds__(kBlock) void reduce_clear_kernel(uint4 *__restrict__ table, size_t n16, uint32_t *__restrict__ counters) {
   const uint4 ones = make_uint4(0xffffffffu, 0xffffffffu, 0xffffffffu, 0xffffffffu);
   for (size_t i = (size_t)blockIdx.x * kBlock + threadIdx.x; i < n16; i += (size_t)gridDim.x * kBlock) table[i] = ones;
@@ -797,14 +909,15 @@
   return check_launch("reduce_onepass");
 }
 
-extern "C" int pynqs_reduce_contract(int64_t nbatch, int sorb, int nele, int noA, int noB, int dtype, int eps_sample,
-                                     const pynqs_reduce_io *io, const double *psi_unique, const double *psi_table, int psi_is_complex,
-                                     int divide, double *eloc, double *psi_x, void *stream) {
+extern "C" int pynqs_reduce_contract_form(int64_t nbatch, int sorb, int nele, int noA, int noB, int dtype, int eps_sample,
+                                          const pynqs_reduce_io *io, const double *psi_unique, const double *psi_table, int psi_is_complex,
+                                          int divide, double *eloc, double *psi_x, int form, void *stream) {
   pynqs::DeviceScope device_scope_(eloc);
   SDParams p;
   if (!make_sd_params(sorb, nele, noA, noB, &p)) return set_error(PYNQS_EINVAL, "bad sorb/noA/noB");
   if (nbatch < 0 || nbatch > 0x7fffffffll || (dtype != PYNQS_F32 && dtype != PYNQS_F64) || eps_sample < 0 || eps_sample > 65535)
     return set_error(PYNQS_EINVAL, "bad nbatch/dtype/eps_sample");
+  if (form != PYNQS_CONTRACT_BATCHED && form != PYNQS_CONTRACT_SERIAL) return set_error(PYNQS_EINVAL, "bad form");
   if (nbatch == 0) return PYNQS_OK;
   if (!io || !io->rec_col || !io->rec_w || !io->rec_link || !io->seg_count || !psi_unique || !eloc || !psi_x ||
       (eps_sample > 0 && (!io->srec_col || !io->srec_w || !io->srec_link)) || (io->lut_table && !psi_table))
@@ -814,15 +927,28 @@
   const int len = (sorb - 1) / 64 + 1;
   hipStream_t st = (hipStream_t)stream;
   const uint32_t grid = (uint32_t)((nbatch + kBlock / 64 - 1) / (kBlock / 64));
-#define PYNQS_CT_LAUNCH(TT, CX)                                                                                                          \
-  hipLaunchKernelGGL((reduce_contract_kernel<TT, CX>), dim3(grid), dim3(kBlock), 0, st, nbatch, nchunks, fixed, (uint32_t)io->cap_doubles, \
-                     (uint32_t)eps_sample, io->rec_col, (const TT *)io->rec_w, io->rec_link, io->seg_count, io->srec_col,                \
-                     (const TT *)io->srec_w, io->srec_link, (const int32_t *)io->dedup_table, dedup_slot_words(len) * 2,                 \
-                     dedup_row_offset(len), (uint32_t)io->cap_unique, psi_unique, psi_table, divide, eloc, psi_x)
+#define PYNQS_CT_ARGS(TT)                                                                                                           \
+  dim3(grid), dim3(kBlock), 0, st, nbatch, nchunks, fixed, (uint32_t)io->cap_doubles, (uint32_t)eps_sample, io->rec_col,            \
+      (const TT *)io->rec_w, io->rec_link, io->seg_count, io->srec_col, (const TT *)io->srec_w, io->srec_link,                      \
+      (const int32_t *)io->dedup_table, dedup_slot_words(len) * 2, dedup_row_offset(len), (uint32_t)io->cap_unique, psi_unique,     \
+      psi_table, divide, eloc, psi_x
+#define PYNQS_CT_LAUNCH(TT, CX)                                                                             \
+  do {                                                                                                      \
+    if (form == PYNQS_CONTRACT_SERIAL) hipLaunchKernelGGL((reduce_contract_kernel<TT, CX>), PYNQS_CT_ARGS(TT)); \
+    else hipLaunchKernelGGL((reduce_contract_batched_kernel<TT, CX, kContractBatch>), PYNQS_CT_ARGS(TT));   \
+  } while (0)
   if (dtype == PYNQS_F64) { if (psi_is_complex) PYNQS_CT_LAUNCH(double, true); else PYNQS_CT_LAUNCH(double, false); }
   else { if (psi_is_complex) PYNQS_CT_LAUNCH(float, true); else PYNQS_CT_LAUNCH(float, false); }
 #undef PYNQS_CT_LAUNCH
+#undef PYNQS_CT_ARGS
   return check_launch("reduce_contract");
+}
+
+extern "C" int pynqs_reduce_contract(int64_t nbatch, int sorb, int nele, int noA, int noB, int dtype, int eps_sample,
+                                     const pynqs_reduce_io *io, const double *psi_unique, const double *psi_table, int psi_is_complex,
+                                     int divide, double *eloc, double *psi_x, void *stream) {
+  return pynqs_reduce_contract_form(nbatch, sorb, nele, noA, noB, dtype, eps_sample, io, psi_unique, psi_table, psi_is_complex, divide, eloc,
+                                    psi_x, PYNQS_CONTRACT_BATCHED, stream);
 }
 
 #ifdef PYNQS_OP_STAMPS
diff --git a/pynqs_amd/grad.py b/pynqs_amd/grad.py
--- a/pynqs_amd/grad.py
+++ b/pynqs_amd/grad.py
@@ -159,6 +159,7 @@
         self.loss = self.flat[o:o + 1]
         self.work = None
         self.events = None
+        self.schedule, self.block = 0, 0
 
     @property
     def params(self):
@@ -193,11 +194,12 @@
         gw, ghb, gvb = self.views
         ws = get_world_size()
         loss_out = torch.empty(1, dtype=torch.float64, device=dev) if ws == 1 else None
-        N.check(N.lib().pynqs_rbm_grad_loss(onv.contiguous().data_ptr(), n, self.sorb, W.data_ptr(), hb.data_ptr(), vb.data_ptr(), self.H,
-                                            self.flavour, prob.data_ptr(), el.data_ptr(), int(cplx), et.data_ptr(),
-                                            pw.data_ptr() if pw is not None else None, gw.data_ptr(), ghb.data_ptr(), gvb.data_ptr(),
-                                            self.loss.data_ptr(), loss_out.data_ptr() if loss_out is not None else None, self.work.data_ptr(),
-                                            torch.cuda.current_stream(dev).cuda_stream), "pynqs_rbm_grad_loss")
+        N.check(N.lib().pynqs_rbm_grad_loss_form(onv.contiguous().data_ptr(), n, self.sorb, W.data_ptr(), hb.data_ptr(), vb.data_ptr(), self.H,
+                                                 self.flavour, prob.data_ptr(), el.data_ptr(), int(cplx), et.data_ptr(),
+                                                 pw.data_ptr() if pw is not None else None, gw.data_ptr(), ghb.data_ptr(), gvb.data_ptr(),
+                                                 self.loss.data_ptr(), loss_out.data_ptr() if loss_out is not None else None,
+                                                 self.work.data_ptr(), self.schedule, self.block,
+                                                 torch.cuda.current_stream(dev).cuda_stream), "pynqs_rbm_grad_loss_form")
         ev = None
         if self.events is not None:
             ev = [torch.cuda.Event(enable_timing=True) for _ in range(2)]
diff --git a/pynqs_amd/reduce_front.py b/pynqs_amd/reduce_front.py
--- a/pynqs_amd/reduce_front.py
+++ b/pynqs_amd/reduce_front.py
@@ -158,7 +158,7 @@
                 "pynqs_reduce_onepass")
 
     def contract(self, values_unique: Tensor, values_table: Optional[Tensor] = None, divide: bool = True,
-                 rec_w: Optional[Tensor] = None, srec_w: Optional[Tensor] = None) -> Tuple[Tensor, Tensor]:
+                 rec_w: Optional[Tensor] = None, srec_w: Optional[Tensor] = None, form: int = 0) -> Tuple[Tensor, Tensor]:
         cplx = values_unique.is_complex()
         vt = torch.complex128 if cplx else torch.float64
         vu = values_unique.to(vt).contiguous()
@@ -170,9 +170,9 @@
         ax = torch.empty(self.n, dtype=vt, device=self.device)
         code = N.PYNQS_F64 if (rec_w if rec_w is not None else self.rec_w).dtype == torch.float64 else N.PYNQS_F32
         st = torch.cuda.current_stream(self.device).cuda_stream
-        N.check(N.lib().pynqs_reduce_contract(self.n, self.sorb, self.nele, self.noa, self.nob, code, self.eps_sample, C.byref(io),
-                                              vu.data_ptr(), tb.data_ptr() if tb is not None else None, int(cplx), int(divide),
-                                              out.data_ptr(), ax.data_ptr(), st), "pynqs_reduce_contract")
+        N.check(N.lib().pynqs_reduce_contract_form(self.n, self.sorb, self.nele, self.noa, self.nob, code, self.eps_sample, C.byref(io),
+                                                   vu.data_ptr(), tb.data_ptr() if tb is not None else None, int(cplx), int(divide),
+                                                   out.data_ptr(), ax.data_ptr(), int(form), st), "pynqs_reduce_contract_form")
         return out, ax
 
     def counters_host(self) -> Tuple[int, int, int]:
```
